# sinamalakouti/CDDMSL

Hardware: AMD Instinct MI355X
Metric: images/sec (train step) VOC+Clipart RN50-C4 (higher is better)
Workload: dtype bf16

## Files before the change

cddmsl_amd/csrc/conv_fwd.hip:

```cpp
#include "gemm_common.h"

namespace {

template <typename T> __device__ __forceinline__ void load8(const char* p, float* f);
template <> __device__ __forceinline__ void load8<__bf16>(const char* p, float* f) {
  const u32x4 v = *(const u32x4*)p;
#pragma unroll
  for (int j = 0; j < 4; ++j) { f[2 * j] = bf2f(v[j] & 0xffff); f[2 * j + 1] = bf2f(v[j] >> 16); }
}
template <> __device__ __forceinline__ void load8<float>(const char* p, float* f) {
  const f32x4 a = ((const f32x4*)p)[0], b = ((const f32x4*)p)[1];
  f[0] = a[0]; f[1] = a[1]; f[2] = a[2]; f[3] = a[3]; f[4] = b[0]; f[5] = b[1]; f[6] = b[2]; f[7] = b[3];
}

__device__ __forceinline__ int swz(int row, int chunk) { return row * KCH + (chunk ^ ((row >> 1) & 7)); }

template <typename T>
__global__ __launch_bounds__(256, 2) void k_conv_fwd_reg(ConvArgs p) {
  __shared__ __attribute__((aligned(16))) u32x4 lds[2][BM * KCH];
  const int t = threadIdx.x;
  const int ntn = (p.Cout + BN - 1) / BN;
  const int tile_n = blockIdx.x % ntn, tile_m = blockIdx.x / ntn;
  const int m0 = tile_m * BM, n0 = tile_n * BN;
  const int cc = t & 7, rb = t >> 3;
// ... 403 lines not shown
            }
#pragma unroll
            for (int j = 0; j < 8; ++j) v[j] += rv[j];
          }
          if (p.relu) {
#pragma unroll
            for (int j = 0; j < 8; ++j) v[j] = fmaxf(v[j], 0.f);
          }
          if (p.relu_mask) {
            float mv[8];
            if (PRE) {
#pragma unroll
              for (int j = 0; j < 4; ++j) { mv[2 * j] = bf2f(rmsk[a][i][j] & 0xffff); mv[2 * j + 1] = bf2f(rmsk[a][i][j] >> 16); }
            } else load8<T>(p.relu_mask + ((long)m * p.ldm + n) * Mma<T>::ES, mv);
#pragma unroll
            for (int j = 0; j < 8; ++j) if (!(mv[j] > 0.f)) v[j] = 0.f;
          }
          if (p.out_f32 || Mma<T>::ES == 4) {
            f32x4* dst = (f32x4*)(p.y + ((long)m * p.ldy + n) * 4);
            f32x4 o0 = {v[0], v[1], v[2], v[3]}, o1 = {v[4], v[5], v[6], v[7]};
            dst[0] = o0; dst[1] = o1;
          } else {
            u32x4 o = {pack2bf(v[0], v[1]), pack2bf(v[2], v[3]), pack2bf(v[4], v[5]), pack2bf(v[6], v[7])};
            *(u32x4*)(p.y + ((long)m * p.ldy + n) * 2) = o;
          }
        }
      }
    }
    return;
  }
#pragma unroll
  for (int b = 0; b < 2; ++b) {
    int n = n0 + wn * 64 + b * 32 + r;
    if (n >= p.Cout) continue;
    float sc = p.scale ? p.scale[n] : 1.f;
    float bi = p.bias ? p.bias[n] : 0.f;
#pragma unroll
    for (int a = 0; a < 2; ++a) {
#pragma unroll
      for (int g = 0; g < 16; ++g) {
        int m = m0 + wm * 64 + a * 32 + (g & 3) + 8 * (g >> 2) + 4 * h;
        if (m >= p.M) continue;
        float v = affine<T>(acc[a][b][g], sc, bi);
        if (p.residual) v += Mma<T>::load(p.residual + ((long)m * p.ldr + n) * Mma<T>::ES);
        if (p.relu) v = fmaxf(v, 0.f);
        if (p.relu_mask && !(Mma<T>::load(p.relu_mask + ((long)m * p.ldm + n) * Mma<T>::ES) > 0.f)) v = 0.f;
        if (p.out_f32) *(float*)(p.y + ((long)m * p.ldy + n) * 4) = v;
        else Mma<T>::store(p.y + ((long)m * p.ldy + n) * Mma<T>::ES, v);
      }
    }
  }
}

template <typename T, int CPP, int NT, int NTAP = 9>
__global__ __launch_bounds__(256) void k_conv3x3_small(ConvArgs p) {
  constexpr int KC = NTAP * CPP, KS = (KC + 1) / 2;
  constexpr int PAD = NTAP == 9 ? 1 : 0;
  constexpr int ES = Mma<T>::ES;
  const int lane = threadIdx.x & 63, r = lane & 31, hh = lane >> 5;
  constexpr bool WLDS = CPP > 1;
  __shared__ __attribute__((aligned(16))) u32x4 wl[WLDS ? NT * KS * 64 : 1];
  u32x4 bw[WLDS ? 1 : NT][WLDS ? 1 : KS];
  {
    const int wv = threadIdx.x >> 6;
#pragma unroll
    for (int nt = 0; nt < NT; ++nt)
#pragma unroll
      for (int ks = 0; ks < KS; ++ks) {
        if (WLDS && ((nt * KS + ks) & 3) != wv) continue;
        const int q = 2 * ks + hh;
        u32x4 v = {0u, 0u, 0u, 0u};
        if (q < KC) v = *(const u32x4*)(p.w + ((long)(nt * 32 + r) * KC + q) * 16);
        if (WLDS) wl[(nt * KS + ks) * 64 + lane] = v;
        else bw[WLDS ? 0 : nt][WLDS ? 0 : ks] = v;
      }
    if (WLDS) __syncthreads();
  }
  float sc[NT], bi[NT];
#pragma unroll
  for (int nt = 0; nt < NT; ++nt) { sc[nt] = p.scale ? p.scale[nt * 32 + r] : 1.f; bi[nt] = p.bias ? p.bias[nt * 32 + r] : 0.f; }
  const int wave = (blockIdx.x * blockDim.x + threadIdx.x) >> 6, nwaves = (gridDim.x * blockDim.x) >> 6;
  const int ntiles = (p.M + 31) >> 5;
  const __amdgpu_buffer_rsrc_t rx = __builtin_amdgcn_make_buffer_rsrc((void*)(p.x - (long)(p.Wi + 1) * (CPP * 16)), 0, 0x7fffffff, 0x00020000);
  const long ybytes = (long)p.M * p.ldy * ES, mbytes = (long)p.M * p.ldm * ES;
  const __amdgpu_buffer_rsrc_t ry = __builtin_amdgcn_make_buffer_rsrc((void*)p.y, 0, (int)(ybytes > 0x7fffffffL ? 0x7fffffffL : ybytes), 0x00020000);
  const __amdgpu_buffer_rsrc_t rm = __builtin_amdgcn_make_buffer_rsrc((void*)p.relu_mask, 0, p.relu_mask ? (int)(mbytes > 0x7fffffffL ? 0x7fffffffL : mbytes) : 0, 0x00020000);
  const float relu_floor = p.relu ? 0.f : -__builtin_inff();
  __shared__ __attribute__((aligned(16))) u32x4 ost[ES == 2 ? 4 * 32 * NT * 4 : 1];
  const bool ost_ok = !p.relu_mask && p.ldy == NT * 32 && (long)p.M * NT * 64 < 0x7fffffffL;
  for (int tile = wave; tile < ntiles; tile += nwaves) {
    const int m = tile * 32 + r;
    const bool vm = m < p.M;
    const unsigned mm = vm ? m : 0;
    const unsigned tq = fdiv(mm, p.dWo), ox = mm - tq * p.Wo;
    const unsigned img = fdiv(tq, p.dHo), oy = tq - img * p.Ho;
    const int iy0 = (int)oy * p.stride - PAD, ix0 = (int)ox * p.stride - PAD;
    const unsigned lbase = (unsigned)((((int)img * p.Hi + iy0 + 1) * p.Wi + ix0 + 1) * (CPP * 16)) + (CPP > 1 ? hh * 16 : 0);
    unsigned bad = vm ? 0u : 0x1ffu;
    if (NTAP == 9) {
#pragma unroll
      for (int ky = 0; ky < 3; ++ky)
#pragma unroll
        for (int kx = 0; kx < 3; ++kx)
          if ((unsigned)(iy0 + ky) >= (unsigned)p.Hi || (unsigned)(ix0 + kx) >= (unsigned)p.Wi) bad |= 1u << (3 * ky + kx);
    }
    u32x4 a[KS];
#pragma unroll
    for (int ks = 0; ks < KS; ++ks) {
      const int q0 = 2 * ks, q1 = 2 * ks + 1;
      const int t0 = q0 / CPP, c0 = q0 % CPP, t1 = q1 / CPP, c1 = q1 % CPP;
      if (CPP > 1) {
        const unsigned v = lbase | (__builtin_amdgcn_ubfe(bad, (unsigned)t0, 1u) << 31);
        a[ks] = __builtin_amdgcn_raw_buffer_load_b128(rx, v, ((t0 / 3) * p.Wi + (t0 % 3)) * (CPP * 16) + c0 * 16, 0);
      } else {
        const int ky = hh ? t1 / 3 : t0 / 3, kx = hh ? t1 % 3 : t0 % 3, cc = hh ? c1 : c0;
        const bool inq = hh ? (q1 < KC) : (q0 < KC);
        const int iy = iy0 + ky, ix = ix0 + kx;
        const bool ok = vm && inq && (unsigned)iy < (unsigned)p.Hi && (unsigned)ix < (unsigned)p.Wi;
        u32x4 v = {0u, 0u, 0u, 0u};
        if (ok) v = *(const u32x4*)(p.x + ((((long)img * p.Hi + iy0) * p.Wi + ix0) + (long)ky * p.Wi + kx) * (CPP * 16) + cc * 16);
        a[ks] = v;
      }
    }
    f32x16 acc[NT];
#pragma unroll
    for (int nt = 0; nt < NT; ++nt)
#pragma unroll
      for (int g = 0; g < 16; ++g) acc[nt][g] = 0.f;
    int wlane = lane;
    asm volatile("" : "+v"(wlane));
#pragma unroll
    for (int ks = 0; ks < KS; ++ks)
#pragma unroll
      for (int nt = 0; nt < NT; ++nt) {
        if (WLDS) Mma<T>::step(acc[nt], a[ks], wl[(nt * KS + ks) * 64 + wlane]);
        else Mma<T>::step(acc[nt], a[ks], bw[WLDS ? 0 : nt][WLDS ? 0 : ks]);
      }
    if (ES == 2 && ost_ok) {
      char* ob = (char*)ost + (threadIdx.x >> 6) * (32 * NT * 64);
#pragma unroll
      for (int nt = 0; nt < NT; ++nt)
#pragma unroll
        for (int g = 0; g < 16; ++g) {
          const int row = (g & 3) + 8 * (g >> 2) + 4 * hh;
          float v = affine<T>(acc[nt][g], sc[nt], bi[nt]);
          asm("v_max_f32 %0, %1, %2" : "=v"(v) : "v"(v), "s"(relu_floor));
          *(unsigned short*)(ob + row * (NT * 64) + (nt * 32 + r) * 2) = f2bf(v);
        }
#pragma unroll
      for (int i = 0; i < 2 * NT; ++i) {
        const u32x4 o = *(const u32x4*)(ob + (i * 64 + lane) * 16);
        __builtin_amdgcn_raw_buffer_store_b128(o, ry, (unsigned)((i * 64 + lane) * 16), tile * (32 * NT * 64), 0);
      }
      continue;
    }
    const unsigned vy = (unsigned)(((tile * 32 + 4 * hh) * p.ldy + r) * ES), vmk = (unsigned)(((tile * 32 + 4 * hh) * p.ldm + r) * ES);
#pragma unroll
    for (int nt = 0; nt < NT; ++nt)
#pragma unroll
      for (int g = 0; g < 16; ++g) {
        const int row = (g & 3) + 8 * (g >> 2);
        float v = affine<T>(acc[nt][g], sc[nt], bi[nt]);
        asm("v_max_f32 %0, %1, %2" : "=v"(v) : "v"(v), "s"(relu_floor));
        if (p.relu_mask) {
          float mv;
          if (ES == 2) mv = bf2f((unsigned)__builtin_amdgcn_raw_buffer_load_b16(rm, vmk, (row * p.ldm + nt * 32) * ES, 0));
          else mv = __builtin_bit_cast(float, __builtin_amdgcn_raw_buffer_load_b32(rm, vmk, (row * p.ldm + nt * 32) * ES, 0));
          if (!(mv > 0.f)) v = 0.f;
        }
        if (ES == 2) __builtin_amdgcn_raw_buffer_store_b16((unsigned short)f2bf(v), ry, vy, (row * p.ldy + nt * 32) * ES, 0);
        else __builtin_amdgcn_raw_buffer_store_b32(__builtin_bit_cast(unsigned, v), ry, vy, (row * p.ldy + nt * 32) * ES, 0);
      }
  }
}

template <typename T> void launch_small(const ConvArgs& a, unsigned nb, hipStream_t st) {
  if (a.KH == 1 && a.cpp == 8) hipLaunchKernelGGL((k_conv3x3_small<T, 8, 2, 1>), dim3(nb), dim3(256), 0, st, a);
  else if (a.KH == 1) hipLaunchKernelGGL((k_conv3x3_small<T, 32, 2, 1>), dim3(nb), dim3(256), 0, st, a);
  else if (a.cpp == 1 && a.Cout == 32) hipLaunchKernelGGL((k_conv3x3_small<T, 1, 1>), dim3(nb), dim3(256), 0, st, a);
  else if (a.cpp == 1) hipLaunchKernelGGL((k_conv3x3_small<T, 1, 2>), dim3(nb), dim3(256), 0, st, a);
  else if (a.cpp == 8) hipLaunchKernelGGL((k_conv3x3_small<T, 8, 2>), dim3(nb), dim3(256), 0, st, a);
  else if (a.Cout == 32) hipLaunchKernelGGL((k_conv3x3_small<T, 4, 1>), dim3(nb), dim3(256), 0, st, a);
  else hipLaunchKernelGGL((k_conv3x3_small<T, 4, 2>), dim3(nb), dim3(256), 0, st, a);
}

template <typename T> void launch_tile128(const ConvArgs& a, const Plan& p, hipStream_t st) {
  const dim3 grid(p.gx, p.gy);
  switch (p.kernel) {
    case 8: launch_small<T>(a, p.gx, st); break;
    case 2: hipLaunchKernelGGL(k_conv_fwd_reg<T>, grid, dim3(256), 0, st, a); break;
    default: hipLaunchKernelGGL(k_conv_fwd<T>, grid, dim3(256), 0, st, a); break;
  }
}

}

void launch_fwd_tile128(const ConvArgs& a, const Plan& p, Operand op, hipStream_t st) {
  if (op == OP_BF16) launch_tile128<__bf16>(a, p, st);
  else launch_tile128<float>(a, p, st);
}
```

cddmsl_amd/csrc/elementwise.hip:

```cpp
#include "common.h"
#include <stdlib.h>

namespace {

template <typename T> struct Elt;
template <> struct Elt<__bf16> {
  static constexpr int ES = 2, VEC = 8;
  __device__ static __forceinline__ void unpack(const u32x4& v, float* f) {
#pragma unroll
    for (int j = 0; j < 4; ++j) { f[2 * j] = bf2f(v[j] & 0xffff); f[2 * j + 1] = bf2f(v[j] >> 16); }
  }
  __device__ static __forceinline__ u32x4 pack(const float* f) {
    u32x4 v;
#pragma unroll
    for (int j = 0; j < 4; ++j) v[j] = pack2bf(f[2 * j], f[2 * j + 1]);
    return v;
  }
  __device__ static __forceinline__ float ld(const char* p) { return bf2f(*(const unsigned short*)p); }
  __device__ static __forceinline__ void st(char* p, float v) { *(unsigned short*)p = f2bf(v); }
};
template <> struct Elt<float> {
  static constexpr int ES = 4, VEC = 4;
  __device__ static __forceinline__ void unpack(const u32x4& v, float* f) {
    const f32x4 x = __builtin_bit_cast(f32x4, v);
// ... 90 lines not shown
                                int RH, int RW, int top, int left, int S, int Cp,
                                float m0, float m1, float m2, float s0, float s1, float s2) {
  preprocess224_px<T>(img, out, n, h, w, Hp, Wp, RH, RW, top, left, S, Cp, m0, m1, m2, s0, s1, s2);
}
template <typename T>
__global__ void k_preprocess224_batch(PreBatch b, char* out, int n0, int Hp, int Wp, int RH, int RW, int top, int left, int S, int Cp,
                                      float m0, float m1, float m2, float s0, float s1, float s2) {
  const int j = blockIdx.y;
  preprocess224_px<T>(b.img[j], out, n0 + j, b.h[j], b.w[j], Hp, Wp, RH, RW, top, left, S, Cp, m0, m1, m2, s0, s1, s2);
}

template <typename T>
__global__ void k_avgpool2_fwd(const char* x, char* y, int N, int H, int W, int cch) {
  int Ho = H / 2, Wo = W / 2;
  long total = (long)N * Ho * Wo * cch;
  for (long i = (long)blockIdx.x * blockDim.x + threadIdx.x; i < total; i += (long)gridDim.x * blockDim.x) {
    int c = i % cch; long q = i / cch;
    int ox = q % Wo; q /= Wo;
    int oy = q % Ho; int n = q / Ho;
    const u32x4* b = (const u32x4*)x + (((long)n * H + 2 * oy) * W + 2 * ox) * cch + c;
    float a0[8], a1[8], a2[8], a3[8], o[8];
    Elt<T>::unpack(b[0], a0); Elt<T>::unpack(b[cch], a1);
    Elt<T>::unpack(b[(long)W * cch], a2); Elt<T>::unpack(b[(long)W * cch + cch], a3);
#pragma unroll
    for (int j = 0; j < Elt<T>::VEC; ++j) o[j] = ((a0[j] + a1[j]) + (a2[j] + a3[j])) * 0.25f;
    ((u32x4*)y)[i] = Elt<T>::pack(o);
  }
}

template <typename T>
__global__ void k_avgpool2_bwd(const char* dy, const char* mask, const char* add, char* dx, int N, int H, int W, int cch) {
  int Ho = H / 2, Wo = W / 2;
  long total = (long)N * H * W * cch;
  for (long i = (long)blockIdx.x * blockDim.x + threadIdx.x; i < total; i += (long)gridDim.x * blockDim.x) {
    int c = i % cch; long q = i / cch;
    int xx = q % W; q /= W;
    int yy = q % H; int n = q / H;
    float g[8], m[8], a[8], o[8];
    bool in = (yy >> 1) < Ho && (xx >> 1) < Wo;
    if (in) Elt<T>::unpack(((const u32x4*)dy)[(((long)n * Ho + (yy >> 1)) * Wo + (xx >> 1)) * cch + c], g);
    if (mask) Elt<T>::unpack(((const u32x4*)mask)[i], m);
    if (add) Elt<T>::unpack(((const u32x4*)add)[i], a);
#pragma unroll
    for (int j = 0; j < Elt<T>::VEC; ++j) {
      float v = in ? g[j] * 0.25f : 0.f;
      if (add) v += a[j];
      if (mask && !(m[j] > 0.f)) v = 0.f;
      o[j] = v;
    }
    ((u32x4*)dx)[i] = Elt<T>::pack(o);
  }
}

__global__ __launch_bounds__(256) void k_avgpool2_bwd_q8(const char* dy, const char* mask, const char* add, char* dx, int N, int H, int W, int cch,
                                                         char* y8, const float* q8, unsigned* amax8) {
  using T = __bf16;
  const int Ho = H / 2, Wo = W / 2;
  const long total = (long)N * H * W * cch;
  const float s = q8[0];
  unsigned mx = 0u;
  for (long i = (long)blockIdx.x * blockDim.x + threadIdx.x; i < total; i += (long)gridDim.x * blockDim.x) {
    int c = i % cch; long q = i / cch;
    int xx = q % W; q /= W;
    int yy = q % H; int n = q / H;
    float g[8], m[8], a[8], o[8];
    bool in = (yy >> 1) < Ho && (xx >> 1) < Wo;
    if (in) Elt<T>::unpack(((const u32x4*)dy)[(((long)n * Ho + (yy >> 1)) * Wo + (xx >> 1)) * cch + c], g);
    if (mask) Elt<T>::unpack(((const u32x4*)mask)[i], m);
    if (add) Elt<T>::unpack(((const u32x4*)add)[i], a);
#pragma unroll
    for (int j = 0; j < 8; ++j) {
      float v = in ? g[j] * 0.25f : 0.f;
      if (add) v += a[j];
      if (mask && !(m[j] > 0.f)) v = 0.f;
      o[j] = v;
      mx = absmax_bits(mx, v);
    }
    ((u32x4*)dx)[i] = Elt<T>::pack(o);
    const u32x2 o8 = {e4m3x4(o[0] * s, o[1] * s, o[2] * s, o[3] * s), e4m3x4(o[4] * s, o[5] * s, o[6] * s, o[7] * s)};
    ((u32x2*)y8)[i] = o8;
  }
  __shared__ unsigned sm[4];
  mx = wave_max_u(mx);
  if ((threadIdx.x & 63) == 0) sm[threadIdx.x >> 6] = mx;
  __syncthreads();
  if (threadIdx.x == 0) {
    const unsigned a = sm[0] > sm[1] ? sm[0] : sm[1], b = sm[2] > sm[3] ? sm[2] : sm[3];
    atomicMax(amax8 + (blockIdx.x & 63), a > b ? a : b);
  }
}

template <typename T>
__global__ void k_maxpool3s2(const char* x, char* y, int N, int H, int W, int Ho, int Wo, int cch) {
  long total = (long)N * Ho * Wo * cch;
  for (long i = (long)blockIdx.x * blockDim.x + threadIdx.x; i < total; i += (long)gridDim.x * blockDim.x) {
    int c = i % cch; long q = i / cch;
    int ox = q % Wo; q /= Wo;
    int oy = q % Ho; int n = q / Ho;
    float m[8], v[8];
#pragma unroll
    for (int j = 0; j < 8; ++j) m[j] = -INFINITY;
    for (int dy = 0; dy < 3; ++dy) {
      int iy = 2 * oy - 1 + dy;
      if (iy < 0 || iy >= H) continue;
      for (int dx = 0; dx < 3; ++dx) {
        int ix = 2 * ox - 1 + dx;
// ... 376 lines not shown
extern "C" int cddmsl_preprocess_batch(const unsigned char* const* imgs, const int* hs, const int* ws, int N, void* out, int Hp, int Wp,
                                       int Cp, const float* mean3, const float* std3, int div255, int dtype, void* stream) {
  if (N < 0 || Cp < 3 || !imgs || !hs || !ws) return CDDMSL_ERR_ARG;
  for (int j = 0; j < N; ++j) if (hs[j] <= 0 || ws[j] <= 0 || hs[j] > Hp || ws[j] > Wp || !imgs[j]) return CDDMSL_ERR_ARG;
  hipStream_t st = (hipStream_t)stream;
  const long px = (long)Hp * Wp;
  for (int n0 = 0; n0 < N; n0 += PRE_MAX) {
    const int c = N - n0 < PRE_MAX ? N - n0 : PRE_MAX;
    PreBatch b;
    for (int j = 0; j < PRE_MAX; ++j) { const int q = j < c ? j : 0; b.img[j] = imgs[n0 + q]; b.h[j] = hs[n0 + q]; b.w[j] = ws[n0 + q]; }
    DISPATCH(dtype, k_preprocess_batch, <<<dim3((unsigned)((px + 255) / 256), (unsigned)c), dim3(256), 0, st>>>(
        b, (char*)out, n0, Hp, Wp, Cp, mean3[0], mean3[1], mean3[2], std3[0], std3[1], std3[2], div255 ? 255.0f : 1.0f));
  }
  return launch_status();
}
extern "C" int cddmsl_preprocess224_batch(const unsigned char* const* imgs, const int* hs, const int* ws, int N, void* out, int Hp, int Wp,
                                          int RH, int RW, int top, int left, int S, int Cp, const float* mean3, const float* std3,
                                          int dtype, void* stream) {
  if (N < 0 || Cp < 3 || !imgs || !hs || !ws || S <= 0 || top < 0 || left < 0 || top + S > RH || left + S > RW) return CDDMSL_ERR_ARG;
  for (int j = 0; j < N; ++j) if (hs[j] <= 0 || ws[j] <= 0 || hs[j] > Hp || ws[j] > Wp || !imgs[j]) return CDDMSL_ERR_ARG;
  hipStream_t st = (hipStream_t)stream;
  for (int n0 = 0; n0 < N; n0 += PRE_MAX) {
    const int c = N - n0 < PRE_MAX ? N - n0 : PRE_MAX;
    PreBatch b;
    for (int j = 0; j < PRE_MAX; ++j) { const int q = j < c ? j : 0; b.img[j] = imgs[n0 + q]; b.h[j] = hs[n0 + q]; b.w[j] = ws[n0 + q]; }
    DISPATCH(dtype, k_preprocess224_batch, <<<dim3((unsigned)((S * S + 255) / 256), (unsigned)c), dim3(256), 0, st>>>(
        b, (char*)out, n0, Hp, Wp, RH, RW, top, left, S, Cp, mean3[0], mean3[1], mean3[2], std3[0], std3[1], std3[2]));
  }
  return launch_status();
}

extern "C" int cddmsl_avgpool2_fwd(const void* x, void* y, int N, int H, int W, int C, int dtype, void* stream) {
  int es = dtype == 0 ? 2 : 4;
  if ((C * es) % 16 || H < 2 || W < 2) return CDDMSL_ERR_ARG;
  int cch = C * es / 16;
  long total = (long)N * (H / 2) * (W / 2) * cch;
  if (total == 0) return CDDMSL_OK;
  DISPATCH(dtype, k_avgpool2_fwd, <<<dim3(gsz(total)), dim3(256), 0, (hipStream_t)stream>>>((const char*)x, (char*)y, N, H, W, cch));
  return launch_status();
}

extern "C" int cddmsl_avgpool2_bwd(const void* dy, const void* mask, const void* add, void* dx, int N, int H, int W,
                                   int C, int dtype, void* stream) {
  int es = dtype == 0 ? 2 : 4;
  if ((C * es) % 16 || H < 2 || W < 2) return CDDMSL_ERR_ARG;
  int cch = C * es / 16;
  long total = (long)N * H * W * cch;
  if (total == 0) return CDDMSL_OK;
  DISPATCH(dtype, k_avgpool2_bwd, <<<dim3(gsz(total)), dim3(256), 0, (hipStream_t)stream>>>(
      (const char*)dy, (const char*)mask, (const char*)add, (char*)dx, N, H, W, cch));
  return launch_status();
}

extern "C" int cddmsl_avgpool2_bwd_q8(const void* dy, const void* mask, const void* add, void* dx, int N, int H, int W, int C, void* y8,
                                      const float* q8, float* amax8, void* stream) {
  if ((C * 2) % 16 || !y8 || !q8 || !amax8) return CDDMSL_ERR_ARG;
  const int cch = C * 2 / 16;
  const long total = (long)N * H * W * cch;
  if (total == 0) return CDDMSL_OK;
  hipLaunchKernelGGL(k_avgpool2_bwd_q8, dim3(gsz(total, 256, 8192)), dim3(256), 0, (hipStream_t)stream, (const char*)dy, (const char*)mask, (const char*)add,
                     (char*)dx, N, H, W, cch, (char*)y8, q8, (unsigned*)amax8);
  return launch_status();
}

extern "C" int cddmsl_maxpool3s2_fwd(const void* x, void* y, int N, int H, int W, int C, int dtype, void* stream) {
  int es = dtype == 0 ? 2 : 4;
  if ((C * es) % 16 || H < 1 || W < 1) return CDDMSL_ERR_ARG;
  int cch = C * es / 16, Ho = (H - 1) / 2 + 1, Wo = (W - 1) / 2 + 1;
  long total = (long)N * Ho * Wo * cch;
  if (total == 0) return CDDMSL_OK;
  DISPATCH(dtype, k_maxpool3s2, <<<dim3(gsz(total)), dim3(256), 0, (hipStream_t)stream>>>((const char*)x, (char*)y, N, H, W, Ho, Wo, cch));
  return launch_status();
}
extern "C" int cddmsl_upsample_zero2(const void* t, const void* mask, const void* add, void* dx, int N, int H, int W, int C,
                                     int dtype, void* stream) {
  int es = dtype == 0 ? 2 : 4;
  if ((C * es) % 16 || H < 1 || W < 1) return CDDMSL_ERR_ARG;
  int cch = C * es / 16, Ho = (H - 1) / 2 + 1, Wo = (W - 1) / 2 + 1;
  long total = (long)N * H * W * cch;
  if (total == 0) return CDDMSL_OK;
  DISPATCH(dtype, k_upsample_zero2, <<<dim3(gsz(total)), dim3(256), 0, (hipStream_t)stream>>>(
      (const char*)t, (const char*)mask, (const char*)add, (char*)dx, N, H, W, Ho, Wo, cch));
  return launch_status();
}
extern "C" int cddmsl_meanpool_fwd(const void* x, float* y, long K, int P, int C, int dtype, void* stream) {
  if (K < 0 || P <= 0 || C <= 0) return CDDMSL_ERR_ARG;
  if (K == 0) return CDDMSL_OK;
  long n = K * C;
  DISPATCH(dtype, k_meanpool_fwd, <<<dim3((unsigned)((n + 255) / 256)), dim3(256), 0, (hipStream_t)stream>>>((const char*)x, y, K, P, C));
  return launch_status();
}
extern "C" int cddmsl_meanpool_bwd(const float* dy, void* dx, long K, int P, int C, int dtype, void* stream) {
  if (K < 0 || P <= 0 || C <= 0) return CDDMSL_ERR_ARG;
  if (K == 0) return CDDMSL_OK;
  long n = K * P * C;
  DISPATCH(dtype, k_meanpool_bwd, <<<dim3((unsigned)((n + 255) / 256)), dim3(256), 0, (hipStream_t)stream>>>(dy, (char*)dx, K, P, C));
  return launch_status();
}

extern "C" int cddmsl_attn_tokens_fwd(const void* x, const float* pos, void* tok, int K, int P, int TP, int C, int dtype, void* stream) {
  int es = dtype == 0 ? 2 : 4;
  if ((C * es) % 16 || P <= 0 || TP < P + 1) return CDDMSL_ERR_ARG;
  int cch = C * es / 16;
  long total = (long)K * cch;
  if (total == 0) return CDDMSL_OK;
  DISPATCH(dtype, k_attn_tokens_fwd, <<<dim3(gsz(total, 64)), dim3(64), 0, (hipStream_t)stream>>>((const char*)x, pos, (char*)tok, nullptr, K, P, TP, cch));
// ... 102 lines not shown
```

cddmsl_amd/csrc/gemm_common.h:

```cpp
#pragma once
#include "common.h"
#include <cstdlib>

namespace {

constexpr int BM = 128, BN = 128, KCH = 8;

struct FastDiv {
  unsigned mul, shr, d;
};
static inline FastDiv make_fastdiv(unsigned d) {
  FastDiv f;
  f.d = d;
  unsigned s = 0;
  while ((1ull << s) < d) ++s;
  f.shr = s;
  f.mul = (unsigned)(((1ull << 32) * ((1ull << s) - d)) / d + 1);
  return f;
}
__device__ __forceinline__ unsigned fdiv(unsigned n, const FastDiv& f) { return (__umulhi(n, f.mul) + n) >> f.shr; }

template <typename T> __device__ __forceinline__ float affine(float v, float sc, float bi) {
  return sizeof(T) <= 2 ? __builtin_fmaf(v, sc, bi) : v * sc + bi;
}

#ifndef CDDMSL_STORE_AUX
#define CDDMSL_STORE_AUX 2
#endif
#ifndef CDDMSL_LOAD_AUX
#define CDDMSL_LOAD_AUX 0
#endif

struct ConvArgs {
  const char* x;
  const char* w;
  char* y;
  const float* scale;
  const float* bias;
  const char* residual;
  const char* relu_mask;
  int Nimg, Hi, Wi, Cin, Ho, Wo, Cout, KH, KW, stride, pad;
  int ldy, ldr, ldm;
  int relu, out_f32, pool;
  int res_f32;
  int res_pool;
  int M, Kc, cpp;
  FastDiv dWo, dHo, dcpp, dKW;
  int xrs, wrs;
  long bx, bw, by;
  char* y8 = nullptr;
  const float* q8 = nullptr;
  unsigned* amax8 = nullptr;
  float* partial = nullptr;
  int tile0 = 0, ksplits = 1, kper = 0, tile_limit = 0;
  int nt_out = 1;
#ifdef CDDMSL_TILE_STAMPS
  unsigned long long* tstamps = nullptr;
#endif
};

template <typename T> struct Mma;
template <> struct Mma<__bf16> {
  static constexpr int ES = 2;
  __device__ static __forceinline__ void step(f32x16& acc, const u32x4& a, const u32x4& b) {
    acc = __builtin_amdgcn_mfma_f32_32x32x16_bf16(__builtin_bit_cast(bf16x8, a), __builtin_bit_cast(bf16x8, b), acc, 0, 0, 0);
  }
  __device__ static __forceinline__ float load(const char* p) { return bf2f(*(const unsigned short*)p); }
  __device__ static __forceinline__ void store(char* p, float v) { *(unsigned short*)p = f2bf(v); }
};
template <> struct Mma<float> {
  static constexpr int ES = 4;
  __device__ static __forceinline__ void step(f32x16& acc, const u32x4& a, const u32x4& b) {
    const f32x4 fa = __builtin_bit_cast(f32x4, a), fb = __builtin_bit_cast(f32x4, b);
    acc = __builtin_amdgcn_mfma_f32_32x32x2f32(fa[0], fb[0], acc, 0, 0, 0);
    acc = __builtin_amdgcn_mfma_f32_32x32x2f32(fa[1], fb[1], acc, 0, 0, 0);
    acc = __builtin_amdgcn_mfma_f32_32x32x2f32(fa[2], fb[2], acc, 0, 0, 0);
    acc = __builtin_amdgcn_mfma_f32_32x32x2f32(fa[3], fb[3], acc, 0, 0, 0);
  }
  __device__ static __forceinline__ float load(const char* p) { return *(const float*)p; }
  __device__ static __forceinline__ void store(char* p, float v) { *(float*)p = v; }
};
typedef __attribute__((ext_vector_type(8))) int i32x8;

__device__ __forceinline__ int xcd_remap(int bid, int nblk) {
  const int q = nblk >> 3, rem = nblk & 7, x = bid & 7, j = bid >> 3;
  return (x < rem ? x * (q + 1) : rem * (q + 1) + (x - rem) * q) + j;
}

template <typename T> __device__ __forceinline__ u32x4 avg4(const u32x4& a, const u32x4& b, const u32x4& c, const u32x4& d);
template <> __device__ __forceinline__ u32x4 avg4<float>(const u32x4& a, const u32x4& b, const u32x4& c, const u32x4& d) {
  const f32x4 fa = __builtin_bit_cast(f32x4, a), fb = __builtin_bit_cast(f32x4, b);
  const f32x4 fc = __builtin_bit_cast(f32x4, c), fd = __builtin_bit_cast(f32x4, d);
  f32x4 r = ((fa + fb) + (fc + fd)) * 0.25f;
  return __builtin_bit_cast(u32x4, r);
}
template <> __device__ __forceinline__ u32x4 avg4<__bf16>(const u32x4& a, const u32x4& b, const u32x4& c, const u32x4& d) {
  u32x4 r;
#pragma unroll
  for (int j = 0; j < 4; ++j) {
    float lo = (bf2f(a[j] & 0xffff) + bf2f(b[j] & 0xffff)) + (bf2f(c[j] & 0xffff) + bf2f(d[j] & 0xffff));
    float hi = (bf2f(a[j] >> 16) + bf2f(b[j] >> 16)) + (bf2f(c[j] >> 16) + bf2f(d[j] >> 16));
    r[j] = pack2bf(lo * 0.25f, hi * 0.25f);
  }
  return r;
}

__device__ __attribute__((aligned(16))) unsigned int g_zero_page[4] = {0u, 0u, 0u, 0u};
// ... 83 lines not shown
```

cddmsl_amd/csrc/gemm_conv.hip:

```cpp
#include "gemm_common.h"

namespace {

template <typename T>
__device__ __forceinline__ void weight_prep_body(const float* w, const float* scale, char* wf, char* wd, int Cout, int KH, int KW, int Cin,
                                                 long first, long stride) {
  __shared__ float tile[32][33];
  const int taps = KH * KW, nit = (Cin + 31) / 32, nct = (Cout + 31) / 32;
  const long ntiles = (long)nct * taps * nit;
  const int tx = threadIdx.x & 31, ty = threadIdx.x >> 5;
  constexpr int ES = Mma<T>::ES;
  for (long tl = first; tl < ntiles; tl += stride) {
    const int it = (int)(tl % nit); const long q = tl / nit;
    const int tap = (int)(q % taps), ct = (int)(q / taps);
    const int ky = tap / KW, kx = tap % KW;
    __syncthreads();
#pragma unroll
    for (int r = 0; r < 4; ++r) {
      const int co = ct * 32 + ty + 8 * r, ci = it * 32 + tx;
      float v = 0.f;
      if (co < Cout && ci < Cin) {
        const long i = ((long)co * taps + tap) * Cin + ci;
        v = w[i];
        if (wf) Mma<T>::store(wf + i * ES, v);
// ... 117 lines not shown
  if ((Cin * es) % 16 != 0) return CDDMSL_ERR_ARG;
  if (pool && (KH != 1 || KW != 1 || pad != 0 || stride != 1)) return CDDMSL_ERR_ARG;
  a.x = (const char*)x; a.w = (const char*)w; a.y = (char*)y; a.scale = scale; a.bias = bias;
  a.residual = (const char*)residual; a.relu_mask = (const char*)relu_mask;
  a.Nimg = Nimg; a.Hi = Hi; a.Wi = Wi; a.Cin = Cin; a.Cout = Cout; a.KH = KH; a.KW = KW; a.stride = stride; a.pad = pad;
  if (pool) { a.Ho = Hi / 2; a.Wo = Wi / 2; }
  else { a.Ho = (Hi + 2 * pad - KH) / stride + 1; a.Wo = (Wi + 2 * pad - KW) / stride + 1; }
  if (a.Ho <= 0 || a.Wo <= 0) return CDDMSL_ERR_ARG;
  if ((out_f32 & 2) && (!(out_f32 & 1) || !residual || relu_mask || pool)) return CDDMSL_ERR_ARG;
  a.ldy = ldy; a.ldr = ldr; a.ldm = ldm; a.relu = relu; a.out_f32 = out_f32 & 1; a.pool = pool;
  a.res_f32 = (op == OP_BF16 && (out_f32 & 2)) ? 1 : 0;
  a.res_pool = (out_f32 & 4) ? 1 : 0;
  if (a.res_pool && (!residual || (out_f32 & 2) || pool || KH != 1 || KW != 1 || pad != 0 || (long)Nimg * (a.Ho / 2) * (a.Wo / 2) * ldr * es >= (1L << 31) ||
                     (Cout & 7) || (ldy & 7) || (ldr & 7) || (relu_mask && (ldm & 7)))) return CDDMSL_ERR_ARG;
  if (a.res_f32 && ((Cout & 7) || (ldy & 7) || (ldr & 7))) return CDDMSL_ERR_ARG;
  long M = (long)Nimg * a.Ho * a.Wo;
  if (M > 0x7fffff00L) return CDDMSL_ERR_ARG;
  a.M = (int)M; a.cpp = Cin * es / 16; a.Kc = KH * KW * a.cpp;
  a.dWo = make_fastdiv((unsigned)a.Wo); a.dHo = make_fastdiv((unsigned)a.Ho);
  a.dcpp = make_fastdiv((unsigned)a.cpp); a.dKW = make_fastdiv((unsigned)KW);
  a.xrs = a.cpp; a.wrs = a.Kc; a.bx = a.bw = a.by = 0;
#ifdef CDDMSL_TILE_STAMPS
  a.tstamps = g_tile_stamps;
#endif
  if (a.M == 0) return CDDMSL_OK;
  a.nt_out = nt_out_for((long)a.M * Cout * 2);
  if (y8) {
    if (op == OP_F32 || (out_f32 & 1) || ldy != Cout) return CDDMSL_ERR_ARG;
    a.y8 = (char*)y8; a.q8 = q8; a.amax8 = (unsigned*)amax8;
  }
  return CDDMSL_OK;
}

static int conv_fwd_any(Operand op, const void* x, const void* w, void* y, const float* scale, const float* bias,
                        const void* residual, const void* relu_mask, int Nimg, int Hi, int Wi, int Cin,
                        int Cout, int KH, int KW, int stride, int pad, int pool, int ldy, int ldr, int ldm,
                        int relu, int out_f32, void* y8, const float* q8, float* amax8, void* stream) {
  ConvArgs a;
  const int st = fill_conv(a, op, x, w, y, scale, bias, residual, relu_mask, Nimg, Hi, Wi, Cin, Cout, KH, KW, stride, pad, pool, ldy, ldr, ldm,
                           relu, out_f32, y8, q8, amax8);
  if (st != CDDMSL_OK || a.M == 0) return st;
  return run_fwd(a, op, plan_fwd(a, op, 1), stream);
}

extern "C" int cddmsl_conv_fwd(const void* x, const void* w, void* y, const float* scale, const float* bias,
                               const void* residual, const void* relu_mask, int Nimg, int Hi, int Wi, int Cin,
                               int Cout, int KH, int KW, int stride, int pad, int pool, int ldy, int ldr, int ldm,
                               int relu, int out_f32, int dtype, void* stream) {
  if (dtype != 0 && dtype != 1) return CDDMSL_ERR_ARG;
  return conv_fwd_any((Operand)dtype, x, w, y, scale, bias, residual, relu_mask, Nimg, Hi, Wi, Cin, Cout, KH, KW, stride, pad, pool, ldy, ldr, ldm,
                      relu, out_f32, nullptr, nullptr, nullptr, stream);
}

extern "C" int cddmsl_conv_fwd_q8(const void* x, const void* w, void* y, const float* scale, const float* bias,
                                  const void* residual, const void* relu_mask, int Nimg, int Hi, int Wi, int Cin,
                                  int Cout, int KH, int KW, int stride, int pad, int relu, void* y8, const float* q8, float* amax8,
                                  void* stream) {
  if (!y8) return CDDMSL_ERR_ARG;
  return conv_fwd_any(OP_BF16, x, w, y, scale, bias, residual, relu_mask, Nimg, Hi, Wi, Cin, Cout, KH, KW, stride, pad, 0, Cout, Cout, Cout,
                      relu, 0, y8, q8, amax8, stream);
}

extern "C" int cddmsl_conv_fwd_fp8(const void* x, const void* w, void* y, const float* scale, const float* bias,
                                   const void* residual, const void* relu_mask, int Nimg, int Hi, int Wi, int Cin, int Cout, int KH,
                                   int KW, int pad, int relu, int out_f32, void* y8, const float* q8, float* amax8, void* stream) {
  if (Cin % 128 != 0 || (out_f32 & ~1)) return CDDMSL_ERR_ARG;
  return conv_fwd_any(OP_FP8, x, w, y, scale, bias, residual, relu_mask, Nimg, Hi, Wi, Cin, Cout, KH, KW, 1, pad, 0, Cout, Cout, Cout,
                      relu, out_f32, y8, q8, amax8, stream);
}

static bool wgrad256_ok(const WgradArgs& a, int batch) {
  const long mode = env_int("CDDMSL_GEMM256", 1);
  if (mode == 0) return false;
  if ((a.Cout & 255) || (a.K & 255) || (a.cpp & 7) || (a.ldd & 7)) return false;
  if (mode == 2) return true;
  return (long)(a.Cout / 256) * (a.K / 256) * batch * ((a.M + WM - 1) / WM) >= env_int("CDDMSL_WGRAD256_MIN", 4000);
}
static bool wgrad256_span_ok(int mtiles_per_split, int Wi, long row_bytes) {
  return ((long)mtiles_per_split * WM + WM + 2L * Wi + 2) * row_bytes + (1L << 20) < (1L << 31);
}

static int even_split(int total_mt, long* splits) {
  const int mps = (int)((total_mt + *splits - 1) / *splits);
  *splits = (total_mt + mps - 1) / mps;
  return mps;
}

static long split_512_rounds(long tiles, int total_mt, bool taps) {
  bool forced;
  const long target = env_int("CDDMSL_WGRAD_BLOCKS", taps ? 1024 : 512, &forced);
  const long maxs = (total_mt + 7) / 8;
  long splits = 1;
  const long r0 = (target + 511) / 512;
  double best = -1.0;
  for (long r = r0; r <= r0 + 1; ++r) {
    long c = (512 * r) / tiles;
    if (c < 1) c = 1;
    if (c > maxs) c = maxs;
    long real = c;
    even_split(total_mt, &real);
    const long blocks = tiles * real, rounds = (blocks + 511) / 512;
    const double eff = (double)blocks / (512.0 * rounds);
    if (eff > best + 0.03) { best = eff; splits = c; }
    if (c == maxs) break;
  }
  if (forced) { splits = (target + tiles - 1) / tiles; if (splits > maxs) splits = maxs; }
// ... 219 lines not shown
```

cddmsl_amd/csrc/losses.hip:

```cpp
#include "common.h"

namespace {

__device__ __forceinline__ float block_sum(float v, float* red) {
  v = wave_sum(v);
  __syncthreads();
  if ((threadIdx.x & 63) == 0) red[threadIdx.x >> 6] = v;
  __syncthreads();
  float s = 0.f;
  for (int i = 0; i < (int)(blockDim.x >> 6); ++i) s += red[i];
  return s;
}
__device__ __forceinline__ float block_max(float v, float* red) {
  v = wave_max(v);
  __syncthreads();
  if ((threadIdx.x & 63) == 0) red[threadIdx.x >> 6] = v;
  __syncthreads();
  float s = -INFINITY;
  for (int i = 0; i < (int)(blockDim.x >> 6); ++i) s = fmaxf(s, red[i]);
  return s;
}

__global__ void k_l2norm_fwd(const float* x, float* y, float* inv, int D, float eps) {
  __shared__ float red[4];
// ... 148 lines not shown
  long tot = (long)n * n;
  k_contrastive_grad<<<dim3((unsigned)((tot + 255) / 256)), dim3(256), 0, (hipStream_t)stream>>>(S, rlse, clse, gloss, dS, n, ld);
  return launch_status();
}

namespace {

template <typename T> struct OutT;
template <> struct OutT<__bf16> { __device__ static __forceinline__ void st(void* p, long i, float v) { ((unsigned short*)p)[i] = f2bf(v); }
                                  __device__ static __forceinline__ float ld(const void* p, long i) { return bf2f(((const unsigned short*)p)[i]); } };
template <> struct OutT<float> { __device__ static __forceinline__ void st(void* p, long i, float v) { ((float*)p)[i] = v; }
                                 __device__ static __forceinline__ float ld(const void* p, long i) { return ((const float*)p)[i]; } };
__device__ __forceinline__ void st4(__bf16*, void* p, long i4, float4 v) { ((uint2*)p)[i4] = make_uint2(pack2bf(v.x, v.y), pack2bf(v.z, v.w)); }
__device__ __forceinline__ void st4(float*, void* p, long i4, float4 v) { ((float4*)p)[i4] = v; }
__device__ __forceinline__ float4 ld4(__bf16*, const void* p, long i4) {
  const uint2 u = ((const uint2*)p)[i4];
  return make_float4(__uint_as_float(u.x << 16), __uint_as_float(u.x & 0xffff0000u), __uint_as_float(u.y << 16), __uint_as_float(u.y & 0xffff0000u));
}
__device__ __forceinline__ float4 ld4(float*, const void* p, long i4) { return ((const float4*)p)[i4]; }

template <typename T, int NSEG>
__global__ __launch_bounds__(256) void k_layernorm_fwd_v(const float* __restrict__ x, const float* __restrict__ gamma,
                                                         const float* __restrict__ beta, void* __restrict__ y, float* __restrict__ mean,
                                                         float* __restrict__ rstd, long R, float eps) {
  constexpr int D = NSEG * 256;
  const long r = (long)blockIdx.x * 4 + (threadIdx.x >> 6);
  const int lane = threadIdx.x & 63;
  if (r >= R) return;
  const float4* xr = (const float4*)(x + r * D);
  float4 v[NSEG];
#pragma unroll
  for (int s = 0; s < NSEG; ++s) v[s] = xr[s * 64 + lane];
  float sum = 0.f;
#pragma unroll
  for (int s = 0; s < NSEG; ++s) sum += (v[s].x + v[s].y) + (v[s].z + v[s].w);
  const float mu = wave_sum(sum) / (float)D;
  float var = 0.f;
#pragma unroll
  for (int s = 0; s < NSEG; ++s) {
    const float a = v[s].x - mu, b = v[s].y - mu, c = v[s].z - mu, d = v[s].w - mu;
    var += (a * a + b * b) + (c * c + d * d);
  }
  const float rs = rsqrtf(wave_sum(var) / (float)D + eps);
#pragma unroll
  for (int s = 0; s < NSEG; ++s) {
    const float4 g = ((const float4*)gamma)[s * 64 + lane], b = ((const float4*)beta)[s * 64 + lane];
    float4 o;
    o.x = (v[s].x - mu) * rs * g.x + b.x; o.y = (v[s].y - mu) * rs * g.y + b.y;
    o.z = (v[s].z - mu) * rs * g.z + b.z; o.w = (v[s].w - mu) * rs * g.w + b.w;
    st4((T*)nullptr, y, r * (D / 4) + s * 64 + lane, o);
  }
  if (lane == 0) { mean[r] = mu; rstd[r] = rs; }
}
template <typename T, int NSEG>
__global__ __launch_bounds__(256) void k_layernorm_bwd_v(const void* __restrict__ dy, const float* __restrict__ x,
                                                         const float* __restrict__ gamma, const float* __restrict__ mean,
                                                         const float* __restrict__ rstd, float* dx, long R, int accumulate) {
  constexpr int D = NSEG * 256;
  const long r = (long)blockIdx.x * 4 + (threadIdx.x >> 6);
  const int lane = threadIdx.x & 63;
  if (r >= R) return;
  const float4* xr = (const float4*)(x + r * D);
  float4* dxr = (float4*)(dx + r * D);
  const float mu = mean[r], rs = rstd[r];
  float4 g[NSEG], xh[NSEG], o[NSEG];
#pragma unroll
  for (int s = 0; s < NSEG; ++s) {
    const float4 d4 = ld4((T*)nullptr, dy, r * (D / 4) + s * 64 + lane), ga = ((const float4*)gamma)[s * 64 + lane], xv = xr[s * 64 + lane];
    if (accumulate) o[s] = dxr[s * 64 + lane];
    g[s] = make_float4(d4.x * ga.x, d4.y * ga.y, d4.z * ga.z, d4.w * ga.w);
    xh[s] = make_float4((xv.x - mu) * rs, (xv.y - mu) * rs, (xv.z - mu) * rs, (xv.w - mu) * rs);
  }
  float sg = 0.f, sgx = 0.f;
#pragma unroll
  for (int s = 0; s < NSEG; ++s) {
    sg += (g[s].x + g[s].y) + (g[s].z + g[s].w);
    sgx += (g[s].x * xh[s].x + g[s].y * xh[s].y) + (g[s].z * xh[s].z + g[s].w * xh[s].w);
  }
  sg = wave_sum(sg) / (float)D; sgx = wave_sum(sgx) / (float)D;
#pragma unroll
  for (int s = 0; s < NSEG; ++s) {
    float4 v;
    v.x = rs * (g[s].x - sg - xh[s].x * sgx); v.y = rs * (g[s].y - sg - xh[s].y * sgx);
    v.z = rs * (g[s].z - sg - xh[s].z * sgx); v.w = rs * (g[s].w - sg - xh[s].w * sgx);
    if (accumulate) { v.x = o[s].x + v.x; v.y = o[s].y + v.y; v.z = o[s].z + v.z; v.w = o[s].w + v.w; }
    dxr[s * 64 + lane] = v;
  }
}
template <typename T> bool layernorm_fwd_v(const float* x, const float* gamma, const float* beta, void* y, float* mean, float* rstd,
                                           long R, int D, float eps, hipStream_t st) {
  const dim3 grid((unsigned)((R + 3) / 4)), blk(256);
  switch (D) {
    case 256: k_layernorm_fwd_v<T, 1><<<grid, blk, 0, st>>>(x, gamma, beta, y, mean, rstd, R, eps); return true;
    case 512: k_layernorm_fwd_v<T, 2><<<grid, blk, 0, st>>>(x, gamma, beta, y, mean, rstd, R, eps); return true;
    case 768: k_layernorm_fwd_v<T, 3><<<grid, blk, 0, st>>>(x, gamma, beta, y, mean, rstd, R, eps); return true;
    case 1024: k_layernorm_fwd_v<T, 4><<<grid, blk, 0, st>>>(x, gamma, beta, y, mean, rstd, R, eps); return true;
  }
  return false;
}
template <typename T> bool layernorm_bwd_v(const void* dy, const float* x, const float* gamma, const float* mean, const float* rstd,
                                           float* dx, long R, int D, int accumulate, hipStream_t st) {
  const dim3 grid((unsigned)((R + 3) / 4)), blk(256);
  switch (D) {
    case 256: k_layernorm_bwd_v<T, 1><<<grid, blk, 0, st>>>(dy, x, gamma, mean, rstd, dx, R, accumulate); return true;
    case 512: k_layernorm_bwd_v<T, 2><<<grid, blk, 0, st>>>(dy, x, gamma, mean, rstd, dx, R, accumulate); return true;
    case 768: k_layernorm_bwd_v<T, 3><<<grid, blk, 0, st>>>(dy, x, gamma, mean, rstd, dx, R, accumulate); return true;
    case 1024: k_layernorm_bwd_v<T, 4><<<grid, blk, 0, st>>>(dy, x, gamma, mean, rstd, dx, R, accumulate); return true;
  }
  return false;
}
__host__ inline bool aligned16(const void* a, const void* b, const void* c, const void* d, const void* e = nullptr) {
  return ((((size_t)a) | ((size_t)b) | ((size_t)c) | ((size_t)d) | ((size_t)e)) & 15) == 0;
}

template <typename T>
__global__ void k_layernorm_fwd(const float* x, const float* gamma, const float* beta, void* y, float* mean, float* rstd,
                                long R, int D, float eps) {
  long r = (long)blockIdx.x * 4 + (threadIdx.x >> 6);
  int lane = threadIdx.x & 63;
  if (r >= R) return;
  const float* xr = x + r * D;
  float s = 0.f;
  for (int d = lane; d < D; d += 64) s += xr[d];
  float mu = wave_sum(s) / (float)D;
  float v = 0.f;
  for (int d = lane; d < D; d += 64) { float c = xr[d] - mu; v += c * c; }
  float rs = rsqrtf(wave_sum(v) / (float)D + eps);
  for (int d = lane; d < D; d += 64) OutT<T>::st(y, r * D + d, (xr[d] - mu) * rs * gamma[d] + beta[d]);
  if (lane == 0) { mean[r] = mu; rstd[r] = rs; }
}
template <typename T>
__global__ void k_layernorm_bwd(const void* dy, const float* x, const float* gamma, const float* mean, const float* rstd,
                                float* dx, long R, int D, int accumulate) {
  long r = (long)blockIdx.x * 4 + (threadIdx.x >> 6);
  int lane = threadIdx.x & 63;
  if (r >= R) return;
  const float* xr = x + r * D;
  float mu = mean[r], rs = rstd[r];
  float sg = 0.f, sgx = 0.f;
  for (int d = lane; d < D; d += 64) {
    float g = OutT<T>::ld(dy, r * D + d) * gamma[d];
    float xh = (xr[d] - mu) * rs;
    sg += g; sgx += g * xh;
  }
  sg = wave_sum(sg) / (float)D; sgx = wave_sum(sgx) / (float)D;
  for (int d = lane; d < D; d += 64) {
    float g = OutT<T>::ld(dy, r * D + d) * gamma[d];
    float xh = (xr[d] - mu) * rs;
    float v = rs * (g - sg - xh * sgx);
    dx[r * D + d] = accumulate ? dx[r * D + d] + v : v;
  }
}

__global__ void k_focal_ce_fwd(const float* logits, const long* target, float* row_loss, float* probs, long R, int C,
                               float gamma, int bg_class, float bg_weight) {
// ... 10 lines not shown
  float zt = __shfl(z, t, 64), pt = __shfl(p, t, 64);
  if (lane == 0) {
    float ce = (mx + logf(se)) - zt;
    float w = (t == bg_class) ? bg_weight : 1.f;
    float mod = gamma > 0.f ? powf(fmaxf(1.f - pt, 0.f), gamma) : 1.f;
    row_loss[r] = ce * mod * w;
  }
}
__global__ void k_focal_ce_bwd(const float* logits, const long* target, const float* probs, const float* gscale, float* dlogits,
                               long R, int C, float gamma, int bg_class, float bg_weight) {
  long r = (long)blockIdx.x * 4 + (threadIdx.x >> 6);
  int lane = threadIdx.x & 63;
  if (r >= R) return;
  int t = (int)target[r];
  float p = lane < C ? probs[r * C + lane] : 0.f;
  float pt = __shfl(p, t, 64);
  float w = (t == bg_class) ? bg_weight : 1.f;
  float one = lane == t ? 1.f : 0.f;
  float ce = -logf(fmaxf(pt, 1e-38f));
  float omp = fmaxf(1.f - pt, 0.f);
  float mod = gamma > 0.f ? powf(omp, gamma) : 1.f;
  float dmod = (gamma > 0.f && omp > 0.f) ? -gamma * powf(omp, gamma - 1.f) * pt * (one - p) : 0.f;
  float g = w * (mod * (p - one) + ce * dmod) * gscale[0];
  if (lane < C) dlogits[r * C + lane] = g;
}

}

extern "C" int cddmsl_layernorm_fwd(const float* x, const float* gamma, const float* beta, void* y, float* mean, float* rstd,
                                    long R, int D, float eps, int dtype, void* stream) {
  if (R < 0 || D <= 0 || (dtype != 0 && dtype != 1)) return CDDMSL_ERR_ARG;
  if (R == 0) return CDDMSL_OK;
  dim3 grid((unsigned)((R + 3) / 4));
  if (aligned16(x, gamma, beta, y) &&
      (dtype == 0 ? layernorm_fwd_v<__bf16>(x, gamma, beta, y, mean, rstd, R, D, eps, (hipStream_t)stream)
                  : layernorm_fwd_v<float>(x, gamma, beta, y, mean, rstd, R, D, eps, (hipStream_t)stream)))
    return launch_status();
  if (dtype == 0) k_layernorm_fwd<__bf16><<<grid, dim3(256), 0, (hipStream_t)stream>>>(x, gamma, beta, y, mean, rstd, R, D, eps);
  else k_layernorm_fwd<float><<<grid, dim3(256), 0, (hipStream_t)stream>>>(x, gamma, beta, y, mean, rstd, R, D, eps);
  return launch_status();
}
extern "C" int cddmsl_layernorm_bwd(const void* dy, const float* x, const float* gamma, const float* mean, const float* rstd,
                                    float* dx, long R, int D, int accumulate, int dtype, void* stream) {
  if (R < 0 || D <= 0 || (dtype != 0 && dtype != 1)) return CDDMSL_ERR_ARG;
  if (R == 0) return CDDMSL_OK;
  dim3 grid((unsigned)((R + 3) / 4));
  if (aligned16(dy, x, gamma, dx) &&
      (dtype == 0 ? layernorm_bwd_v<__bf16>(dy, x, gamma, mean, rstd, dx, R, D, accumulate, (hipStream_t)stream)
                  : layernorm_bwd_v<float>(dy, x, gamma, mean, rstd, dx, R, D, accumulate, (hipStream_t)stream)))
    return launch_status();
  if (dtype == 0) k_layernorm_bwd<__bf16><<<grid, dim3(256), 0, (hipStream_t)stream>>>(dy, x, gamma, mean, rstd, dx, R, D, accumulate);
  else k_layernorm_bwd<float><<<grid, dim3(256), 0, (hipStream_t)stream>>>(dy, x, gamma, mean, rstd, dx, R, D, accumulate);
  return launch_status();
}
extern "C" int cddmsl_focal_ce_fwd(const float* logits, const long* target, float* row_loss, float* probs, long R, int C,
                                   float gamma, int bg_class, float bg_weight, void* stream) {
  if (R < 0 || C <= 0 || C > 64) return CDDMSL_ERR_ARG;
  if (R == 0) return CDDMSL_OK;
  k_focal_ce_fwd<<<dim3((unsigned)((R + 3) / 4)), dim3(256), 0, (hipStream_t)stream>>>(logits, target, row_loss, probs, R, C, gamma, bg_class, bg_weight);
  return launch_status();
}
extern "C" int cddmsl_focal_ce_bwd(const float* logits, const long* target, const float* probs, const float* gscale,
                                   float* dlogits, long R, int C, float gamma, int bg_class, float bg_weight, void* stream) {
  if (R < 0 || C <= 0 || C > 64) return CDDMSL_ERR_ARG;
  if (R == 0) return CDDMSL_OK;
  k_focal_ce_bwd<<<dim3((unsigned)((R + 3) / 4)), dim3(256), 0, (hipStream_t)stream>>>(logits, target, probs, gscale, dlogits, R, C, gamma, bg_class, bg_weight);
  return launch_status();
}

namespace {
struct BoxW { float wx, wy, ww, wh; };
__device__ __forceinline__ void get_deltas4(const float* s, const float* t, BoxW w, float* d) {
  const float sw = s[2] - s[0], sh = s[3] - s[1];
  const float sx = s[0] + 0.5f * sw, sy = s[1] + 0.5f * sh;
  const float tw = t[2] - t[0], th = t[3] - t[1];
  const float tx = t[0] + 0.5f * tw, ty = t[1] + 0.5f * th;
  d[0] = w.wx * (tx - sx) / sw; d[1] = w.wy * (ty - sy) / sh;
  d[2] = w.ww * logf(tw / sw); d[3] = w.wh * logf(th / sh);
}
__device__ __forceinline__ float sgn(float v) { return v > 0.f ? 1.f : (v < 0.f ? -1.f : 0.f); }

__global__ __launch_bounds__(256) void k_rpn_losses(const float* logits, const float* deltas, const long* pos, int npos, const long* neg, int nneg,
                                                     const long* midx, const float* gt, const long* gt_off, const float* anchors, long A, BoxW w,
                                                     float inv_norm, float* out2, const float* gout2, float* dlogits, float* ddeltas) {
  __shared__ float red[4];
  const bool bwd = gout2 != nullptr;
  const float gc = bwd ? gout2[0] * inv_norm : 0.f, gl = bwd ? gout2[1] * inv_norm : 0.f;
  float cls = 0.f, loc = 0.f;
  for (int i = threadIdx.x; i < npos + nneg; i += blockDim.x) {
    const bool is_pos = i < npos;
    const long r = is_pos ? pos[i] : neg[i - npos];
    const float x = logits[r], y = is_pos ? 1.f : 0.f;
    if (!bwd) cls += fmaxf(x, 0.f) - x * y + log1pf(expf(-fabsf(x)));
    else dlogits[r] = (1.f / (1.f + expf(-x)) - y) * gc;
    if (is_pos) {
      const long img = r / A, a = r - img * A;
      float d[4];
      get_deltas4(anchors + 4 * a, gt + 4 * (midx[r] + gt_off[img]), w, d);
#pragma unroll
      for (int c = 0; c < 4; ++c) {
        const float e = deltas[4 * r + c] - d[c];
        if (!bwd) loc += fabsf(e); else ddeltas[4 * r + c] = sgn(e) * gl;
      }
    }
  }
  if (!bwd) {
// ... 46 lines not shown
```

cddmsl_amd/hip.py:

```python
import ctypes
import os
from ctypes import c_float, c_int, c_long, c_void_p

import torch

from ._lib import check, lib, ptr, require_cuda, stream_ptr

DT = {torch.bfloat16: 0, torch.float32: 1}

_sigs_done = False


def _L():
    global _sigs_done
    L = lib()
    if not _sigs_done:
        vp, ci, cf = c_void_p, c_int, c_float
        L.cddmsl_last_kernel.argtypes = []
        L.cddmsl_plan_only.argtypes = [ci]
        L.cddmsl_conv_fwd.argtypes = [vp] * 7 + [ci] * 16 + [vp]
        L.cddmsl_bottleneck64_ok.argtypes = [ci] * 4
        L.cddmsl_bottleneck64_fwd.argtypes = [vp] * 17 + [ci] * 4 + [vp]
        L.cddmsl_conv_wgrad.argtypes = [vp] * 4 + [ci] * 12 + [vp]
        L.cddmsl_set_workspace.argtypes = [vp, c_long]
        L.cddmsl_weight_prep.argtypes = [vp] * 4 + [ci] * 5 + [vp]
        L.cddmsl_weight_prep_multi.argtypes = [vp, ci, ci, vp]
        L.cddmsl_preprocess.argtypes = [vp, vp] + [ci] * 6 + [vp, vp, ci, ci, vp]
        L.cddmsl_maxpool3s2_fwd.argtypes = [vp, vp] + [ci] * 5 + [vp]
        L.cddmsl_upsample_zero2.argtypes = [vp] * 4 + [ci] * 5 + [vp]
        L.cddmsl_meanpool_fwd.argtypes = [vp, vp, c_long, ci, ci, ci, vp]
        L.cddmsl_meanpool_bwd.argtypes = [vp, vp, c_long, ci, ci, ci, vp]
        L.cddmsl_preprocess224.argtypes = [vp, vp] + [ci] * 11 + [vp, vp, ci, vp]
        L.cddmsl_preprocess_batch.argtypes = [vp, vp, vp, ci, vp, ci, ci, ci, vp, vp, ci, ci, vp]
        L.cddmsl_preprocess224_batch.argtypes = [vp, vp, vp, ci, vp] + [ci] * 8 + [vp, vp, ci, vp]
        L.cddmsl_avgpool2_fwd.argtypes = [vp, vp] + [ci] * 5 + [vp]
        L.cddmsl_avgpool2_bwd.argtypes = [vp] * 4 + [ci] * 5 + [vp]
        L.cddmsl_avgpool2_bwd_q8.argtypes = [vp] * 4 + [ci] * 4 + [vp] * 4
        L.cddmsl_attn_tokens_fwd.argtypes = [vp] * 3 + [ci] * 5 + [vp]
        L.cddmsl_attn_tokens_bwd.argtypes = [vp] * 4 + [ci] * 5 + [vp]
        L.cddmsl_attnpool_softmax_fwd.argtypes = [vp] * 3 + [c_long, ci, ci, ci, cf, ci, vp]
        L.cddmsl_attnpool_softmax_bwd.argtypes = [vp] * 4 + [c_long, ci, ci, ci, cf, ci, vp]
        L.cddmsl_gemm_nt_batched.argtypes = [vp] * 4 + [ci] * 7 + [c_long] * 3 + [ci, ci, vp]
        L.cddmsl_gemm_tn_batched.argtypes = [vp] * 3 + [ci] * 7 + [c_long] * 3 + [ci, ci, vp]
        L.cddmsl_relu_bwd.argtypes = [vp, vp, vp, c_long, ci, ci, vp]
        L.cddmsl_colsum.argtypes = [vp, vp, c_long, ci, ci, ci, vp]
        L.cddmsl_sgd_clip_step.argtypes = [vp] * 4 + [ci, vp] + [cf] * 4 + [ci, vp]
        L.cddmsl_roi_align_forward.argtypes = [vp] * 5 + [ci] * 7 + [cf, ci, ci, ci, vp]
        L.cddmsl_roi_align_backward.argtypes = [vp] * 7 + [ci] * 7 + [cf, ci, ci, ci, vp]
        L.cddmsl_nms_anyorder.argtypes = [vp] * 4 + [ci, cf, vp, vp, vp]
        L.cddmsl_roi_align_nchw_anyorder.argtypes = [vp] * 3 + [ci] * 7 + [cf, ci, ci, ci, vp, vp, vp]
        L.cddmsl_roi_align_backward_nchw_anyorder.argtypes = [vp] * 3 + [ci] * 7 + [cf, ci, ci, ci, vp, vp, vp]
        L.cddmsl_quantize_fp8.argtypes = [vp] * 4 + [c_long, ci, vp]
        L.cddmsl_conv_fwd_fp8.argtypes = [vp] * 7 + [ci] * 10 + [vp] * 4
        L.cddmsl_conv_wgrad_fp8_ok.argtypes = [ci] * 6
        L.cddmsl_conv_wgrad_fp8.argtypes = [vp] * 4 + [ci] * 9 + [vp]
        L.cddmsl_conv_fwd_q8.argtypes = [vp] * 7 + [ci] * 10 + [vp] * 4
        L.cddmsl_fp8_dot_nt.argtypes = [vp] * 4 + [ci] * 4 + [vp]
        L.cddmsl_roi_align_forward_affine.argtypes = [vp] * 6 + [ci] * 8 + [cf, ci, ci, ci] + [vp] * 4
        L.cddmsl_roi_align_backward_pooled.argtypes = [vp] * 7 + [ci] * 7 + [cf, ci, ci, ci, vp]
        L.cddmsl_anchors.argtypes = [vp, vp, ci, ci, ci, cf, cf, vp]
        L.cddmsl_sort_desc.argtypes = [vp] * 5 + [ci, ci, vp, vp, vp]
        L.cddmsl_rpn_decode.argtypes = [vp] * 6 + [ci] * 5 + [cf] * 8 + [vp]
        L.cddmsl_nms.argtypes = [vp] * 5 + [ci, ci, cf, ci, vp]
        L.cddmsl_iou_match.argtypes = [vp, ci, vp, ci, vp, vp, vp, ci, cf, cf, ci, ci, ci, ci, vp]
        L.cddmsl_iou_match_batched.argtypes = [vp] * 7 + [ci] * 5 + [cf, cf] + [ci] * 4 + [vp]
        L.cddmsl_l2norm_fwd.argtypes = [vp, vp, vp, c_long, ci, cf, vp]
        L.cddmsl_l2norm_bwd.argtypes = [vp, vp, vp, vp, c_long, ci, vp]
        L.cddmsl_cosine_logits_fwd.argtypes = [vp] * 4 + [c_long, ci, ci, cf, cf, vp]
        L.cddmsl_cosine_logits_bwd.argtypes = [vp] * 5 + [c_long, ci, ci, cf, ci, vp]
        L.cddmsl_layernorm_fwd.argtypes = [vp] * 6 + [c_long, ci, cf, ci, vp]
        L.cddmsl_layernorm_bwd.argtypes = [vp] * 6 + [c_long, ci, ci, ci, vp]
        L.cddmsl_focal_ce_fwd.argtypes = [vp] * 4 + [c_long, ci, cf, ci, cf, vp]
        L.cddmsl_focal_ce_bwd.argtypes = [vp] * 5 + [c_long, ci, cf, ci, cf, vp]
        L.cddmsl_attn_small_fwd.argtypes = [vp] * 4 + [ci] * 8 + [cf, ci, vp]
        L.cddmsl_attn_small_bwd.argtypes = [vp] * 7 + [ci] * 8 + [cf, ci, vp]
        L.cddmsl_attn_tokens_fwd_mask.argtypes = [vp] * 4 + [ci] * 5 + [vp]
        L.cddmsl_attnpool_dx.argtypes = [vp] * 6 + [ci] * 6 + [vp]
        L.cddmsl_rpn_losses.argtypes = [vp, vp, vp, ci, vp, ci, vp, vp, vp, vp, c_long, cf, cf, cf, cf, cf, vp, vp, vp, vp, vp]
        L.cddmsl_box_l1.argtypes = [vp, ci, vp, ci, vp, vp, vp, cf, cf, cf, cf, cf, vp, vp, vp, vp]
        L.cddmsl_attn_last_fwd.argtypes = [vp] * 4 + [ci] * 8 + [cf, ci, vp]
        L.cddmsl_attn_last_bwd.argtypes = [vp] * 6 + [ci] * 8 + [cf, ci, vp]
        L.cddmsl_contrastive_fwd.argtypes = [vp] * 4 + [ci, ci, vp]
        L.cddmsl_contrastive_bwd.argtypes = [vp] * 5 + [ci, ci, vp]
        L.cddmsl_instance_boxes.argtypes = [vp] + [ci] * 4 + [vp, ci, vp, vp, vp, vp]
        L.cddmsl_text_embed.argtypes = [vp] * 4 + [c_long, ci, ci, ci, ci, vp]
        L.cddmsl_attn_causal_fwd.argtypes = [vp, vp] + [ci] * 6 + [cf, ci, vp]
        L.cddmsl_quick_gelu.argtypes = [vp, c_long, ci, vp]
        L.cddmsl_text_pool.argtypes = [vp] * 5 + [c_long, ci, ci, ci, cf, ci, vp]
        L.cddmsl_skinny_gemm_workspace.argtypes = [ci] * 3
        L.cddmsl_skinny_gemm.argtypes = [vp] * 6 + [c_long] + [ci] * 4 + [vp]
        L.cddmsl_lm_head_workspace.argtypes = [ci, ci]
        L.cddmsl_lm_head_argmax.argtypes = [vp, vp, vp, ci, vp, vp, c_long, ci, ci, ci, vp]
        L.cddmsl_decode_attn.argtypes = [vp] * 4 + [ci] * 6 + [cf, ci, vp]
        L.cddmsl_pos_embed.argtypes = [vp, ci] + [vp] * 4 + [c_long] + [ci] * 6 + [vp]
        L.cddmsl_gelu_new.argtypes = [vp, c_long, ci, vp]
        L.cddmsl_lm_head_topk_workspace.argtypes = [ci, ci]
        L.cddmsl_lm_head_topk.argtypes = [vp] * 7 + [c_long] + [ci] * 4 + [vp]
        L.cddmsl_beam_step.argtypes = [vp] * 15 + [ci] * 5 + [vp]
        L.cddmsl_decode_attn_beam.argtypes = [vp] * 7 + [ci] * 9 + [cf, ci, vp]
        _sigs_done = True
    return L


class _Profiler:

    def __init__(self):
        self.on = False
        self.only = None
        self.events = []
        self.shapes = []

    def enable(self, only=None):
        self.on, self.only, self.events, self.shapes = True, (set(only) if only else None), [], []

    def begin(self, name=None, plan=None):
        if not self.on:
            return None
        if self.only is not None:
            if name is None and plan is not None:
                L = _L()
                L.cddmsl_plan_only(1)
                try:
                    plan()
                finally:
# ... 84 lines not shown
    N, H, W, Cin = x.shape
    Cout, KH, KW, Cin2 = w.shape
    assert Cin == Cin2, (x.shape, w.shape)
    if pool:
        Ho, Wo = H // 2, W // 2
    else:
        Ho, Wo = (H + 2 * pad - KH) // stride + 1, (W + 2 * pad - KW) // stride + 1
    ydt = torch.float32 if out_f32 else x.dtype
    if out_spec is not None and out_spec.full is None:
        out_spec.full = torch.empty((2 * N, Ho, Wo, Cout), device=x.device, dtype=ydt)
        y, out_spec.used = out_spec.full[:N], 1
    elif out_spec is not None and out_spec.used == 1 and tuple(out_spec.full.shape) == (2 * N, Ho, Wo, Cout) and out_spec.full.dtype == ydt:
        y, out_spec.used = out_spec.full[N:], 2
    else:
        y = torch.empty((N, Ho, Wo, Cout), device=x.device, dtype=ydt)
    for v in (scale, bias):
        assert v is None or (v.dtype == torch.float32 and v.numel() == Cout and v.is_contiguous())
    res_f32 = residual is not None and residual.dtype == torch.float32 and x.dtype != torch.float32
    if res_f32:
        assert out_f32 and relu_mask is None and not pool and Cout % 8 == 0
    if residual_pooled:
        assert residual is not None and not res_f32 and residual.dtype == x.dtype and residual.is_contiguous()
        assert tuple(residual.shape) == (N, Ho // 2, Wo // 2, Cout) and pooled_residual_ok(residual), residual.shape
    for v in (residual, relu_mask):
        assert v is None or (v is residual and residual_pooled) or (
            (v.dtype == x.dtype or (v is residual and res_f32)) and v.is_contiguous() and v.numel() == y.numel())
    y8 = None
    if emit8 is not None:
        assert x.dtype == torch.bfloat16 and not out_f32 and not pool and not residual_pooled and not res_f32
        y8 = torch.empty(y.shape, device=x.device, dtype=torch.uint8)

    def launch():
        if y8 is not None:
            return _L().cddmsl_conv_fwd_q8(ptr(x), ptr(w), ptr(y), ptr(scale), ptr(bias), ptr(residual), ptr(relu_mask),
                                           N, H, W, Cin, Cout, KH, KW, stride, pad, int(relu), ptr(y8), ptr(emit8[0]), ptr(emit8[1]), stream_ptr())
        return _L().cddmsl_conv_fwd(ptr(x), ptr(w), ptr(y), ptr(scale), ptr(bias), ptr(residual), ptr(relu_mask),
                                    N, H, W, Cin, Cout, KH, KW, stride, pad, int(pool), Cout, Cout, Cout,
                                    int(relu), int(out_f32) | (2 if res_f32 else 0) | (4 if residual_pooled else 0), _dt(x), stream_ptr())
    e0 = PROFILE.begin(plan=launch) if PROFILE.on else None
    st = launch()
    check(st, "cddmsl_conv_fwd")
    PROFILE.end(e0, _CONV_KERNEL.get(_L().cddmsl_last_kernel(), "conv_fwd") if e0 is not None else "conv_fwd",
                2.0 * N * Ho * Wo * Cout * KH * KW * Cin,
                (N * Ho * Wo, Cout, KH * KW * Cin, KH, int(pool), stride),
                nbytes=float(_conv_input_pixels(N, H, W, Ho, Wo, KH, KW, stride, bool(pool)) * Cin * x.element_size()
                             + w.numel() * w.element_size() + y.numel() * y.element_size()
                             + (residual.numel() * residual.element_size() if residual is not None else 0)
                             + (relu_mask.numel() * relu_mask.element_size() if relu_mask is not None else 0)))
    if y8 is not None:
        y._fp8 = (y8, emit8[0].data_ptr())
    return y


def bottleneck64_ok(o1, w2, w3, wd=None, w1n=None):
    if not (o1.is_cuda and o1.dtype == torch.bfloat16 and o1.dim() == 4 and o1.is_contiguous() and o1.shape[3] == 64):
        return False
    want = ((w2, (64, 3, 3, 64)), (w3, (256, 1, 1, 64)), (wd, (256, 1, 1, 64)), (w1n, (64, 1, 1, 256)))
    if any(w is not None and (tuple(w.shape) != s or w.dtype != torch.bfloat16 or not w.is_contiguous()) for w, s in want):
        return False
    N, H, W, _ = o1.shape
    return N > 0 and bool(_L().cddmsl_bottleneck64_ok(N, H, W, 0))


def bottleneck64_fwd(o1, w2, bn2, w3, bn3, residual=None, x0=None, wd=None, bnd=None, w1n=None, bn1n=None):
    require_cuda(o1, w2, w3, residual, x0, wd, w1n)
    assert bottleneck64_ok(o1, w2, w3, wd, w1n) and (residual is None) != (wd is None)
    N, H, W, _ = o1.shape
    for t, c in ((residual, 256), (x0 if wd is not None else None, 64)):
        assert t is None or (t.dtype == torch.bfloat16 and t.is_contiguous() and tuple(t.shape) == (N, H, W, c))
    for bn, c in ((bn2, 64), (bn3, 256), (bnd, 256), (bn1n, 64)):
        assert bn is None or all(v.dtype == torch.float32 and v.numel() == c and v.is_contiguous() and v.is_cuda for v in bn)
    assert (wd is None) == (bnd is None) and (w1n is None) == (bn1n is None) and (wd is None or x0 is not None)
    out = torch.empty((N, H, W, 256), device=o1.device, dtype=o1.dtype)
    o1n = torch.empty((N, H, W, 64), device=o1.device, dtype=o1.dtype) if w1n is not None else None
    sd, bd = bnd if bnd is not None else (None, None)
    s1n, b1n = bn1n if bn1n is not None else (None, None)
    e0 = PROFILE.begin(name="k_bottleneck64") if PROFILE.on else None
    check(_L().cddmsl_bottleneck64_fwd(ptr(o1), ptr(w2), ptr(bn2[0]), ptr(bn2[1]), ptr(w3), ptr(bn3[0]), ptr(bn3[1]), ptr(residual),
                                       ptr(x0 if wd is not None else None), ptr(wd), ptr(sd), ptr(bd), ptr(w1n), ptr(s1n), ptr(b1n),
                                       ptr(out), ptr(o1n), N, H, W, 0, stream_ptr()), "cddmsl_bottleneck64_fwd")
    M = N * H * W
    kn = 576 * 64 + 64 * 256 + (64 * 256 if wd is not None else 0) + (256 * 64 if w1n is not None else 0)
    PROFILE.end(e0, "k_bottleneck64", 2.0 * M * kn, (M, 256, 576, 3, int(wd is not None), int(w1n is not None)),
                nbytes=float(2 * M * (64 + (64 if wd is not None else 256) + 256 + (64 if w1n is not None else 0)) + 2 * kn))
    return out, o1n


def conv_emit8_ok(M, Cout, KH, KW, Cin_chunks_ok=True):
    return Cout % 256 == 0 and KH * KW <= 31 and ((M + 255) // 256) * (Cout // 256) >= 160 and Cin_chunks_ok and os.environ.get("CDDMSL_GEMM256", "1") != "0"


FP8_MAX = 448.0


@_timed("quantize_fp8")
def quantize_fp8(x, scale=None, amax=None):
    require_cuda(x, scale, amax)
    assert x.is_contiguous() and x.dtype in (torch.bfloat16, torch.float32) and x.numel() % 8 == 0
    y = torch.empty(x.shape, device=x.device, dtype=torch.uint8)
    check(_L().cddmsl_quantize_fp8(ptr(x), ptr(y), ptr(scale), ptr(amax), x.numel(), 0 if x.dtype == torch.bfloat16 else 1, stream_ptr()),
          "cddmsl_quantize_fp8")
    return y


def conv_fwd_fp8_ok(M, Cin, Cout, KH, KW, pad):
    min_tiles = int(os.environ.get("CDDMSL_FP8_MIN_TILES", "160"))
# ... 142 lines not shown
def _f3(v):
    return (c_float * 3)(*[float(x) for x in v])


def _image_table(images_u8):
    import ctypes
    n = len(images_u8)
    ptrs = (ctypes.c_void_p * n)(*[im.data_ptr() for im in images_u8])
    hs = (ctypes.c_int * n)(*[int(im.shape[1]) for im in images_u8])
    ws = (ctypes.c_int * n)(*[int(im.shape[2]) for im in images_u8])
    return ptrs, hs, ws


@_timed("preprocess")
def preprocess(images_u8, Hp, Wp, mean, std, dtype, Cp=None, div255=True):
    require_cuda(*images_u8)
    Cp = Cp or (8 if dtype == torch.bfloat16 else 4)
    out = torch.empty((len(images_u8), Hp, Wp, Cp), device=images_u8[0].device, dtype=dtype)
    m, s = _f3(mean), _f3(std)
    for im in images_u8:
        assert im.dtype == torch.uint8 and im.dim() == 3 and im.shape[0] == 3 and im.is_contiguous()
    ptrs, hs, ws = _image_table(images_u8)
    check(_L().cddmsl_preprocess_batch(ptrs, hs, ws, len(images_u8), ptr(out), Hp, Wp, Cp, m, s, int(div255), DT[dtype], stream_ptr()),
          "cddmsl_preprocess_batch")
    return out


@_timed("preprocess224")
def preprocess224(images_u8, Hp, Wp, mean, std, dtype, size=224, Cp=None):
    require_cuda(*images_u8)
    Cp = Cp or (8 if dtype == torch.bfloat16 else 4)
    if Wp <= Hp:
        RW, RH = size, int(size * Hp / Wp)
    else:
        RH, RW = size, int(size * Wp / Hp)
    top, left = int(round((RH - size) / 2.0)), int(round((RW - size) / 2.0))
    out = torch.empty((len(images_u8), size, size, Cp), device=images_u8[0].device, dtype=dtype)
    m, s = _f3(mean), _f3(std)
    for im in images_u8:
        assert im.dtype == torch.uint8 and im.dim() == 3 and im.is_contiguous()
    ptrs, hs, ws = _image_table(images_u8)
    check(_L().cddmsl_preprocess224_batch(ptrs, hs, ws, len(images_u8), ptr(out), Hp, Wp, RH, RW, top, left, size, Cp,
                                           m, s, DT[dtype], stream_ptr()), "cddmsl_preprocess224_batch")
    return out


@_timed("avgpool2_fwd")
def avgpool2_fwd(x):
    require_cuda(x)
    N, H, W, C = x.shape
    y = torch.empty((N, H // 2, W // 2, C), device=x.device, dtype=x.dtype)
    check(_L().cddmsl_avgpool2_fwd(ptr(x), ptr(y), N, H, W, C, _dt(x), stream_ptr()), "cddmsl_avgpool2_fwd")
    return y


@_timed("avgpool2_bwd")
def avgpool2_bwd(dy, in_shape, mask=None, add=None, emit8=None):
    require_cuda(dy, mask, add)
    N, H, W, C = in_shape
    assert dy.is_contiguous() and tuple(dy.shape) == (N, H // 2, W // 2, C)
    dx = torch.empty(in_shape, device=dy.device, dtype=dy.dtype)
    if emit8 is not None and dy.dtype == torch.bfloat16:
        y8 = torch.empty(in_shape, device=dy.device, dtype=torch.uint8)
        check(_L().cddmsl_avgpool2_bwd_q8(ptr(dy), ptr(mask), ptr(add), ptr(dx), N, H, W, C, ptr(y8), ptr(emit8[0]), ptr(emit8[1]), stream_ptr()),
              "cddmsl_avgpool2_bwd_q8")
        dx._fp8 = (y8, emit8[0].data_ptr())
        return dx
    check(_L().cddmsl_avgpool2_bwd(ptr(dy), ptr(mask), ptr(add), ptr(dx), N, H, W, C, _dt(dy), stream_ptr()), "cddmsl_avgpool2_bwd")
    return dx


@_timed("attn_tokens_fwd")
def attn_tokens_fwd(x, pos, tp=None):
    require_cuda(x, pos)
    K, P, C = x.shape
    tp = tp or P + 1
    assert pos.dtype == torch.float32 and tuple(pos.shape) == (P + 1, C) and x.is_contiguous() and pos.is_contiguous()
    tok = torch.empty((K, tp, C), device=x.device, dtype=x.dtype)
    check(_L().cddmsl_attn_tokens_fwd(ptr(x), ptr(pos), ptr(tok), K, P, tp, C, _dt(x), stream_ptr()), "cddmsl_attn_tokens_fwd")
    return tok


@_timed("attn_tokens_fwd")
def attn_tokens_fwd_mask(x, pos, tp=None):
    require_cuda(x, pos)
    K, P, C = x.shape
    tp = tp or P + 1
    assert pos.dtype == torch.float32 and tuple(pos.shape) == (P + 1, C) and x.is_contiguous() and pos.is_contiguous() and P <= 64
    tok = torch.empty((K, tp, C), device=x.device, dtype=x.dtype)
    mbits = torch.empty((K, C), device=x.device, dtype=torch.int64)
    check(_L().cddmsl_attn_tokens_fwd_mask(ptr(x), ptr(pos), ptr(tok), ptr(mbits), K, P, tp, C, _dt(x), stream_ptr()), "cddmsl_attn_tokens_fwd_mask")
    return tok, mbits


def rpn_losses(logits, deltas, pos, neg, midx, gt, gt_off, anchors, weights, inv_norm, gout=None):
    require_cuda(logits, deltas, pos, neg, midx, gt, gt_off, anchors)
    for t in (logits, deltas, gt, anchors):
        assert t.dtype == torch.float32 and t.is_contiguous()
    for t in (pos, neg, midx, gt_off):
        assert t.dtype == torch.int64 and t.is_contiguous()
    A = anchors.shape[0]
    assert deltas.numel() == 4 * logits.numel() and midx.numel() == logits.numel()
    args = (ptr(logits), ptr(deltas), ptr(pos), pos.numel(), ptr(neg), neg.numel(), ptr(midx), ptr(gt), ptr(gt_off), ptr(anchors), A,
            *[float(w) for w in weights], float(inv_norm))
    if gout is None:
        out = torch.empty(2, device=logits.device, dtype=torch.float32)
# ... 428 lines not shown

def cosine_logits_bwd(ds, x, wn, inv, temperature, dx=None):
    require_cuda(ds, x, wn, inv, dx)
    R, D = x.shape
    ds = ds.contiguous()
    assert x.dtype == wn.dtype == inv.dtype == ds.dtype == torch.float32 and x.is_contiguous() and wn.is_contiguous() and inv.is_contiguous()
    assert wn.dim() == 2 and wn.shape[1] == D and tuple(ds.shape) == (R, wn.shape[0] + 1) and inv.numel() == R
    acc = dx is not None
    if dx is None:
        dx = torch.empty_like(x)
    assert dx.dtype == torch.float32 and dx.is_contiguous() and dx.shape == x.shape
    check(_L().cddmsl_cosine_logits_bwd(ptr(ds), ptr(x), ptr(wn), ptr(inv), ptr(dx), R, D, wn.shape[0], temperature, int(acc),
                                         stream_ptr()), "cddmsl_cosine_logits_bwd")
    return dx


def contrastive_fwd(S):
    require_cuda(S)
    n = S.shape[0]
    assert S.dtype == torch.float32 and S.shape == (n, n) and S.is_contiguous()
    rl = torch.empty(n, device=S.device, dtype=torch.float32)
    cl = torch.empty(n, device=S.device, dtype=torch.float32)
    loss = torch.empty(1, device=S.device, dtype=torch.float32)
    check(_L().cddmsl_contrastive_fwd(ptr(S), ptr(rl), ptr(cl), ptr(loss), n, n, stream_ptr()), "cddmsl_contrastive_fwd")
    return loss, rl, cl


def contrastive_bwd(S, rl, cl, gloss):
    require_cuda(S, rl, cl, gloss)
    n = S.shape[0]
    assert S.dtype == rl.dtype == cl.dtype == torch.float32 and tuple(S.shape) == (n, n) and S.is_contiguous()
    assert rl.is_contiguous() and cl.is_contiguous() and rl.numel() == n and cl.numel() == n and gloss.numel() == 1
    dS = torch.empty_like(S)
    check(_L().cddmsl_contrastive_bwd(ptr(S), ptr(rl), ptr(cl), ptr(gloss.reshape(1).float().contiguous()), ptr(dS), n, n, stream_ptr()),
          "cddmsl_contrastive_bwd")
    return dS


@_timed("layernorm")
def layernorm_fwd(x, gamma, beta, out_dtype, eps=1e-5):
    require_cuda(x, gamma, beta)
    R, D = x.shape
    assert x.dtype == gamma.dtype == beta.dtype == torch.float32 and x.is_contiguous() and gamma.is_contiguous() and beta.is_contiguous()
    assert gamma.numel() == D and beta.numel() == D
    y = torch.empty((R, D), device=x.device, dtype=out_dtype)
    mean = torch.empty(R, device=x.device, dtype=torch.float32)
    rstd = torch.empty(R, device=x.device, dtype=torch.float32)
    check(_L().cddmsl_layernorm_fwd(ptr(x), ptr(gamma), ptr(beta), ptr(y), ptr(mean), ptr(rstd), R, D, eps, DT[out_dtype], stream_ptr()),
          "cddmsl_layernorm_fwd")
    return y, mean, rstd


@_timed("layernorm")
def layernorm_bwd(dy, x, gamma, mean, rstd, accumulate_into=None):
    require_cuda(dy, x, gamma, mean, rstd, accumulate_into)
    R, D = x.shape
    dy = dy.contiguous()
    assert x.dtype == gamma.dtype == mean.dtype == rstd.dtype == torch.float32 and x.is_contiguous() and gamma.is_contiguous()
    assert mean.is_contiguous() and rstd.is_contiguous() and gamma.numel() == D and mean.numel() == R and rstd.numel() == R and dy.shape == x.shape
    if accumulate_into is None:
        dx, acc = torch.empty_like(x), 0
    else:
        assert accumulate_into.dtype == torch.float32 and accumulate_into.is_contiguous() and accumulate_into.shape == x.shape
        dx, acc = accumulate_into, 1
    check(_L().cddmsl_layernorm_bwd(ptr(dy), ptr(x), ptr(gamma), ptr(mean), ptr(rstd), ptr(dx), R, D, acc, _dt(dy), stream_ptr()),
          "cddmsl_layernorm_bwd")
    return dx


def _attn_views(q, kv, t, heads):
    assert q.dim() == 2 and kv.dim() == 2 and q.is_contiguous() and kv.is_contiguous() and q.dtype == kv.dtype == torch.bfloat16
    R, d = q.shape
    assert kv.shape == (R, 2 * d) and R % t == 0 and d % heads == 0
    return R // t, d, d // heads


@_timed("attn_small")
def attn_small_fwd(q, kv, t, heads, scale):
    require_cuda(q, kv)
    n, d, dh = _attn_views(q, kv, t, heads)
    o = torch.empty_like(q)
    vptr = c_void_p(kv.data_ptr() + d * 2)
    check(_L().cddmsl_attn_small_fwd(ptr(q), ptr(kv), vptr, ptr(o), n, t, heads, dh, d, 2 * d, 2 * d, d, float(scale), 0, stream_ptr()),
          "cddmsl_attn_small_fwd")
    return o


@_timed("attn_last")
def attn_last_fwd(q, kv, t, heads, scale):
    require_cuda(q, kv)
    n, d = q.shape
    assert q.dtype == kv.dtype == torch.bfloat16 and q.is_contiguous() and kv.is_contiguous() and tuple(kv.shape) == (n * t, 2 * d)
    o = torch.empty((n, d), device=q.device, dtype=q.dtype)
    p = torch.empty((n, heads, t), device=q.device, dtype=torch.float32)
    check(_L().cddmsl_attn_last_fwd(ptr(q), ptr(kv), ptr(o), ptr(p), n, t, heads, d // heads, d, 2 * d, d, d, float(scale), 0, stream_ptr()),
          "cddmsl_attn_last_fwd")
    return o, p


@_timed("attn_last")
def attn_last_bwd(q, kv, do, p, t, heads, scale):
    require_cuda(q, kv, do, p)
    n, d = q.shape
    do = do.contiguous()
    assert do.shape == (n, d) and do.dtype == q.dtype and p.is_contiguous()
    dq, dkv = torch.empty_like(q), torch.empty_like(kv)
    check(_L().cddmsl_attn_last_bwd(ptr(q), ptr(kv), ptr(do), ptr(p), ptr(dq), ptr(dkv), n, t, heads, d // heads, d, 2 * d, d, d, float(scale), 0,
                                    stream_ptr()), "cddmsl_attn_last_bwd")
    return dq, dkv


@_timed("attn_small")
def attn_small_fwd_qkv(qkv, t, heads, scale):
    require_cuda(qkv)
    assert qkv.dim() == 2 and qkv.is_contiguous() and qkv.dtype == torch.bfloat16 and qkv.shape[1] % 3 == 0 and qkv.shape[0] % t == 0
    R, d = qkv.shape[0], qkv.shape[1] // 3
    o = torch.empty((R, d), device=qkv.device, dtype=qkv.dtype)
# ... 283 lines not shown
```

cddmsl_amd/layers.py:

```python
import os
import weakref

import torch

from . import hip

_STEP = [0]


def bump_weight_version():
    _STEP[0] += 1


_LOAD_GEN = [0]


def note_weights_loaded(*_):
    _LOAD_GEN[0] += 1
    _STEP[0] += 1


def load_generation():
    return _LOAD_GEN[0]

# ... 230 lines not shown
    key = (-1 if pw.frozen else _STEP[0], wd.data_ptr(), pw.param._version, _LOAD_GEN[0])
    c = getattr(pw, "_fp8d", None)
    if c is None or c[0] != key:
        amax = wd.abs().amax().float().clamp_min(1e-20).view(1)
        pw._fp8d = c = (key, hip.quantize_fp8(wd, hip.FP8_MAX / amax), amax / hip.FP8_MAX)
    return c[1], c[2]


def fp8_slot_of(owner, name):
    sl = getattr(owner, name, None)
    dev = (owner.param if hasattr(owner, "param") else owner.w[0]).device
    if sl is None or sl.scale.device != dev:
        sl = FP8_SCALES.slot(dev)
        setattr(owner, name, sl)
    return sl


def dgrad_auto(g, pw, fp8=False, slot=None, emit8=None, **kw):
    T = g.dtype
    _, wd = pw.get(T, True)
    if fp8 and T == torch.bfloat16 and slot is not None and not kw.get("residual_pooled", False):
        Cout_d, KH, KW, Cin_d = wd.shape
        pad = kw.get("pad", 0)
        N, H, W, _ = g.shape
        M = N * (H + 2 * pad - KH + 1) * (W + 2 * pad - KW + 1)
        if hip.conv_fwd_fp8_ok(M, Cin_d, Cout_d, KH, KW, pad):
            g8 = fp8_copy(g, slot)
            wd8, d_w = fp8_weight_d(pw, wd)
            return hip.conv_fwd_fp8(g8, wd8, (slot.deq * d_w).expand(Cout_d).contiguous(), None, kw.get("residual"), False, kw.get("relu_mask"),
                                    pad, emit8=emit8)
    if emit8 is not None:
        Cout_d, KH, KW, Cin_d = wd.shape
        N, H, W, _ = g.shape
        pad = kw.get("pad", 0)
        M = N * (H + 2 * pad - KH + 1) * (W + 2 * pad - KW + 1)
        if not (T == torch.bfloat16 and hip.conv_emit8_ok(M, Cout_d, KH, KW, (Cin_d * 2 // 16) % 8 == 0) and not kw.get("residual_pooled", False)):
            emit8 = None
    return hip.conv_fwd(g, wd, emit8=emit8, **kw)


def _fp8_dgrad_wanted(pw, g_shape, pad, fp8):
    if not fp8:
        return False
    Cout, KH, KW, Cin = _ohwi(pw.param).shape
    N, H, W, _ = g_shape
    M = N * (H + 2 * pad - KH + 1) * (W + 2 * pad - KW + 1)
    return hip.conv_fwd_fp8_ok(M, Cout, Cin, KH, KW, pad)


def cat_prepared(weights, dtype):
    return torch.cat([hip.weight_prep(_ohwi(w.detach()), None, dtype, True, False)[0] for w in weights], dim=0)


class ConvFn(torch.autograd.Function):

    @staticmethod
    def forward(ctx, x, anchor, pw, bias, stride, pad, relu, out_f32, train_w, residual=None, fp8=False):
        y = conv_fwd_auto(x, pw, None, None if bias is None else bias.detach(), fp8, residual=None if residual is None else residual.detach(),
                          relu=relu, stride=stride, pad=pad, out_f32=out_f32)
        ctx.pw, ctx.bias, ctx.cfg = pw, bias, (stride, pad, relu, out_f32, train_w)
        ctx.fp8 = bool(fp8)
        ctx.save_for_backward(x, y if relu else None, _fp8_made_for(x, pw) if fp8 else None)
        return y

    @staticmethod
    def backward(ctx, dy):
        x, y, x8 = ctx.saved_tensors
        stride, pad, relu, out_f32, train_w = ctx.cfg
        f8 = ctx.fp8 and x8 is not None and stride == 1
        g_slot = fp8_slot_of(ctx.pw, "_fp8_g") if f8 else None
        T = x.dtype
        dy_in = dy
        dy = dy.contiguous()
        if relu:
            dy = hip.relu_bwd(dy, y if y.dtype == T else y.to(T))
        elif dy.dtype != T:
            dy = dy.to(T)
        w = ctx.pw.param
        if train_w:
            if f8:
                wgrad_auto(x, dy, ctx.pw, None, pad, _ohwi(_grad_buf(w)), True, x8, g_slot, min_m=65536)
            else:
                hip.conv_wgrad(x, dy, _ohwi(w).shape, None, stride=stride, pad=pad, out=_ohwi(_grad_buf(w)))
            if ctx.bias is not None:
                hip.colsum(dy.view(-1, dy.shape[-1]), out=_grad_buf(ctx.bias))
        dx = None
        if ctx.needs_input_grad[0]:
            assert stride == 1, "input gradient of a strided conv is not on the hot path"
            _, wd = ctx.pw.get(T, need_dgrad=True)
            KH = _ohwi(w).shape[1]
            Kd, rows = dy.shape[-1], dy.numel() // dy.shape[-1]
            if KH == 1 and _ohwi(w).shape[2] == 1 and pad == 0 and rows <= 1024 and Kd >= 8192 and Kd % (16 * 64) == 0:
                S, N = 16, x.shape[-1]
                part = torch.empty(S, rows, N, device=dy.device, dtype=torch.float32)
                hip.gemm_nt_batched(dy, wd, part, rows, N, Kd // S, Kd, Kd, N, S, Kd // S, Kd // S, rows * N)
                dx = part.sum(0).to(T).view(x.shape)
            elif f8:
                dx = dgrad_auto(dy, ctx.pw, True, g_slot, pad=KH - 1 - pad)
            else:
                dx = hip.conv_fwd(dy, wd, stride=1, pad=KH - 1 - pad)
        return dx, None, None, None, None, None, None, None, None, (dy_in if ctx.needs_input_grad[9] else None), None


class FrozenMlpFn(torch.autograd.Function):

    @staticmethod
    def forward(ctx, x, pw1, b1, pw2, b2, residual):
        T = x.dtype
        w1, _ = pw1.get(T, need_dgrad=False)
        w2, _ = pw2.get(T, need_dgrad=False)
        M, K = x.shape
        h = hip.conv_fwd(x.view(1, 1, M, K), w1, None, b1.detach(), relu=True)
        y = hip.conv_fwd(h, w2, None, b2.detach(), residual.detach().view(1, 1, M, -1), out_f32=True)
        ctx.pw = (pw1, pw2)
        ctx.save_for_backward(h)
        return y.view(M, -1)

    @staticmethod
    def backward(ctx, dy):
        (h,) = ctx.saved_tensors
        T = h.dtype
        M = h.shape[2]
        g = dy.contiguous()
        if g.dtype != T:
            g = g.to(T)
        _, w2d = ctx.pw[1].get(T, need_dgrad=True)
        _, w1d = ctx.pw[0].get(T, need_dgrad=True)
        dh = hip.conv_fwd(g.view(1, 1, M, -1), w2d, relu_mask=h)
        dx = hip.conv_fwd(dh, w1d).view(M, -1) if ctx.needs_input_grad[0] else None
        return dx, None, None, None, None, (dy if ctx.needs_input_grad[5] else None)


def frozen_mlp(x2d, pw1, b1, pw2, b2, residual):
    return FrozenMlpFn.apply(x2d.contiguous(), pw1, b1, pw2, b2, residual.contiguous())


def conv(x, pw, bias=None, stride=1, pad=0, relu=False, out_f32=False, train_w=True, residual=None, fp8=False):
    anchor = pw.param if train_w else None
    assert residual is None or not relu
    return ConvFn.apply(x, anchor, pw, bias, stride, pad, relu, out_f32, train_w, residual, fp8)


def linear(x2d, pw, bias=None, relu=False, out_f32=False, train_w=True, residual=None):
    M, K = x2d.shape
    y = conv(x2d.contiguous().view(1, 1, M, K), pw, bias, 1, 0, relu, out_f32, train_w,
             None if residual is None else residual.contiguous().view(1, 1, M, -1))
    return y.view(M, -1)


class FusedHeadsFn(torch.autograd.Function):

    @staticmethod
    def forward(ctx, x, anchor, heads, out_f32):
        T = x.dtype
        K = heads[0][0].shape[1] if heads[0][0].dim() == 2 else heads[0][0].shape[1]
        ws = [w.detach().reshape(w.shape[0], -1) for w, _ in heads]
        n = sum(w.shape[0] for w in ws)
        npad = (n + 7) // 8 * 8
        wcat = torch.zeros(npad, 1, 1, ws[0].shape[1], device=x.device, dtype=torch.float32)
        wcat[:n, 0, 0] = torch.cat(ws, dim=0)
        bcat = torch.zeros(npad, device=x.device, dtype=torch.float32)
        bcat[:n] = torch.cat([b.detach() for _, b in heads])
        wf, wd = hip.weight_prep(wcat, None, T, True, True)
        y = hip.conv_fwd(x, wf, None, bcat, out_f32=out_f32)
        ctx.heads, ctx.wd, ctx.npad = heads, wd, npad
        ctx.save_for_backward(x)
        return y

    @staticmethod
    def backward(ctx, dy):
        (x,) = ctx.saved_tensors
        T = x.dtype
        dy = dy.contiguous()
        if dy.dtype != T:
            dy = dy.to(T)
        K = x.shape[-1]
        dw = hip.conv_wgrad(x, dy, (ctx.npad, 1, 1, K))
        db = hip.colsum(dy.view(-1, ctx.npad))
        off = 0
        for w, b in ctx.heads:
            n = w.shape[0]
            _grad_buf(w).view(n, -1).add_(dw[off:off + n].view(n, -1)) if w.dim() == 2 else \
                _ohwi(_grad_buf(w)).add_(dw[off:off + n])
            _grad_buf(b).add_(db[off:off + n])
            off += n
        dx = hip.conv_fwd(dy, ctx.wd) if ctx.needs_input_grad[0] else None
        return dx, None, None, None


def fused_heads(x, heads, out_f32=True):
    return FusedHeadsFn.apply(x, heads[0][0], heads, out_f32)


class BlockParams:

    def __init__(self, w1, w2, w3, wd, bn1, bn2, bn3, bnd, stride, frozen, fp8=False):
        self.stride, self.frozen, self.fp8 = stride, frozen, fp8
        self.bn = (bn1, bn2, bn3, bnd)
        self.w = (w1, w2, w3, wd)
        self.pw = tuple(None if w is None else PreparedWeight(w, b[0], frozen) for w, b in zip(self.w, self.bn))


def _block_forward(x, bp, save, px_given=None, next_pw=None, out_spec=None):
    (s1, b1), (s2, b2), (s3, b3), bnd = bp.bn
    pool = bp.stride > 1
    f8 = bp.fp8
    o1_shape = (x.shape[0], x.shape[1], x.shape[2], _ohwi(bp.w[0]).shape[0])
    o1 = conv_fwd_auto(x, bp.pw[0], s1, b1, f8, emit8=fp8_emit_for(bp.pw[1], o1_shape, 1, f8), relu=True)
    x8 = _fp8_made_for(x, bp.pw[0]) if f8 and save else None
    M2 = x.shape[0] * x.shape[1] * x.shape[2]
    e8o2 = fp8_act_slot(bp.pw[2]).emit() if save and not pool and _fp8_wgrad1x1_wanted(bp.pw[2], M2, f8) else None
    o2 = conv_fwd_auto(o1, bp.pw[1], s2, b2, f8, emit8=e8o2, relu=True, pad=1)
    o2_8 = _fp8_made_for(o2, bp.pw[2]) if e8o2 is not None else None
    p2 = hip.avgpool2_fwd(o2) if pool else o2
    if pool and px_given is not None and tuple(px_given.shape) == (x.shape[0], x.shape[1] // 2, x.shape[2] // 2, x.shape[3]):
        px = px_given
    else:
        px = hip.avgpool2_fwd(x) if pool else x
    if bp.pw[3] is not None:
        idn = conv_fwd_auto(px, bp.pw[3], bnd[0], bnd[1], f8)
    else:
        idn = x
    out_shape = (p2.shape[0], p2.shape[1], p2.shape[2], _ohwi(bp.w[2]).shape[0])
    out = conv_fwd_auto(p2, bp.pw[2], s3, b3, f8, emit8=fp8_emit_for(next_pw, out_shape, 0, f8), residual=idn, relu=True, out_spec=out_spec)
    return out, ((o1, o2, p2 if pool else None, px if pool else None, (x8, _fp8_made_for(o1, bp.pw[1]) if f8 else None, o2_8)) if save else None)


def _block_backward(gs, x, o1, o2, p2, px, bp, need_dx, mask_x, prev_bp=None, c8=(None, None, None)):
    T = x.dtype
    (s1, _), (s2, _), (s3, _), bnd = bp.bn
    pool = bp.stride > 1
    f8 = bp.fp8 and T == torch.bfloat16
    w1p, w2p, w3p, wdp = bp.w
    shp = lambda w: _ohwi(w).shape
    gs_slot = fp8_slot_of(bp, "_fp8_gs") if f8 else None
    d2_slot = fp8_slot_of(bp.pw[1], "_fp8_g") if f8 else None
    x8, o1_8, o2_8 = c8
    M2 = o2.shape[0] * o2.shape[1] * o2.shape[2]
    if o2_8 is not None and not pool:
        wgrad_auto(o2, gs, bp.pw[2], s3, 0, _ohwi(_grad_buf(w3p)), f8, o2_8, gs_slot, taps_only=False)
    else:
        hip.conv_wgrad(p2 if pool else o2, gs, shp(w3p), s3, out=_ohwi(_grad_buf(w3p)))
    d1_slot = fp8_slot_of(bp.pw[0], "_fp8_g") if f8 and x8 is not None and _fp8_wgrad1x1_wanted(bp.pw[0], M2, f8) else None
    if pool:
        dp2 = dgrad_auto(gs, bp.pw[2], f8, gs_slot)
        dpre2 = hip.avgpool2_bwd(dp2, tuple(o2.shape), mask=o2, emit8=d2_slot.emit() if f8 and _fp8_dgrad_wanted(bp.pw[1], o2.shape, 1, f8) else None)
    else:
        e8 = d2_slot.emit() if f8 and _fp8_dgrad_wanted(bp.pw[1], o2.shape, 1, f8) else None
        dpre2 = dgrad_auto(gs, bp.pw[2], f8, gs_slot, emit8=e8, relu_mask=o2)
    dpre1 = dgrad_auto(dpre2, bp.pw[1], f8, d2_slot, pad=1, relu_mask=o1, emit8=d1_slot.emit() if d1_slot is not None else None)
    wgrad_auto(o1, dpre2, bp.pw[1], s2, 1, _ohwi(_grad_buf(w2p)), f8, o1_8, d2_slot)
    if d1_slot is not None:
        wgrad_auto(x, dpre1, bp.pw[0], s1, 0, _ohwi(_grad_buf(w1p)), f8, x8, d1_slot, taps_only=False)
    else:
        hip.conv_wgrad(x, dpre1, shp(w1p), s1, out=_ohwi(_grad_buf(w1p)))
    if wdp is not None:
        hip.conv_wgrad(px if pool else x, gs, shp(wdp), bnd[0], out=_ohwi(_grad_buf(wdp)))
    if not need_dx:
        return None
    pooled = False
    if wdp is not None:
        dxb = dgrad_auto(gs, bp.pw[3], f8, gs_slot)
        if pool:
            pooled = x.shape[1] % 2 == 0 and x.shape[2] % 2 == 0 and hip.pooled_residual_ok(dxb)
            if not pooled:
                dxb = hip.avgpool2_bwd(dxb, tuple(x.shape))
    else:
        dxb = gs
    e8 = None
    if f8 and prev_bp is not None and prev_bp.fp8 and not pooled and _fp8_dgrad_wanted(prev_bp.pw[2], x.shape, 0, True):
        e8 = fp8_slot_of(prev_bp, "_fp8_gs").emit()
    return dgrad_auto(dpre1, bp.pw[0], False, None, emit8=e8, residual=dxb, relu_mask=x if mask_x else None, residual_pooled=pooled)


class ResStageFn(torch.autograd.Function):
    @staticmethod
    def forward(ctx, x, anchor, blocks, out_grad_premasked=False, px0=None, out_spec=None):
        ctx.out_grad_premasked = out_grad_premasked
        saved, o1_8s = [x], []
        cur = x
        for bi, bp in enumerate(blocks):
            cur, mids = _block_forward(cur, bp, True, px0 if bi == 0 else None, blocks[bi + 1].pw[0] if bi + 1 < len(blocks) else None,
                                       out_spec if bi + 1 == len(blocks) else None)
            saved += [mids[0], mids[1], mids[2], mids[3], cur]
            o1_8s += list(mids[4])
        ctx.blocks = blocks
        ctx.save_for_backward(*saved, *o1_8s)
        return cur

    @staticmethod
    def backward(ctx, g):
        blocks = ctx.blocks
        saved, o1_8s = ctx.saved_tensors[:-3 * len(blocks)], ctx.saved_tensors[-3 * len(blocks):]
        need_dx = ctx.needs_input_grad[0]
        gs = g.contiguous() if ctx.out_grad_premasked else hip.relu_bwd(g.contiguous(), saved[-1])
        for i in range(len(blocks) - 1, -1, -1):
            x, o1, o2, p2, px = saved[5 * i: 5 * i + 5]
            gs = _block_backward(gs, x, o1, o2, p2, px, blocks[i], need_dx or i > 0, mask_x=i > 0, prev_bp=blocks[i - 1] if i > 0 else None,
                                 c8=tuple(o1_8s[3 * i: 3 * i + 3]))
        return gs, None, None, None, None, None


def _fused_stage_ok(x, blocks, out_spec):
    if os.environ.get("CDDMSL_FUSED_BOTTLENECK", "1") == "0" or out_spec is not None:
        return False
    if not (x.is_cuda and x.dtype == torch.bfloat16 and x.dim() == 4 and x.is_contiguous()):
        return False
    cin = x.shape[3]
    for bi, bp in enumerate(blocks):
        if bp.fp8 or bp.stride != 1 or any(v is None for b in bp.bn[:3] for v in b):
            return False
        if tuple(_ohwi(bp.w[0]).shape) != (64, 1, 1, cin) or tuple(_ohwi(bp.w[1]).shape) != (64, 3, 3, 64) or tuple(_ohwi(bp.w[2]).shape) != (256, 1, 1, 64):
            return False
        if bp.w[3] is not None:
            if bi > 0 or cin != 64 or tuple(_ohwi(bp.w[3]).shape) != (256, 1, 1, 64) or any(v is None for v in bp.bn[3]):
                return False
        elif cin != 256:
            return False
        cin = 256
    return bool(blocks) and bool(hip._L().cddmsl_bottleneck64_ok(x.shape[0], x.shape[1], x.shape[2], 0))


def _fused_stage_forward(x, blocks):
    T = x.dtype
    wf = lambda pw: pw.get(T, need_dgrad=False)[0]
    o1 = conv_fwd_auto(x, blocks[0].pw[0], blocks[0].bn[0][0], blocks[0].bn[0][1], False, relu=True)
    cur = x
    for bi, bp in enumerate(blocks):
        nxt = blocks[bi + 1] if bi + 1 < len(blocks) else None
        kw = dict(x0=cur, wd=wf(bp.pw[3]), bnd=bp.bn[3]) if bp.pw[3] is not None else dict(residual=cur)
        if nxt is not None:
            kw.update(w1n=wf(nxt.pw[0]), bn1n=nxt.bn[0])
        cur, o1 = hip.bottleneck64_fwd(o1, wf(bp.pw[1]), bp.bn[1], wf(bp.pw[2]), bp.bn[2], **kw)
    return cur


def res_stage(x, blocks, frozen, out_grad_premasked=False, out_spec=None):
    px0 = getattr(x, "_pooled2", None)
    if frozen or not torch.is_grad_enabled():
        if _fused_stage_ok(x, blocks, out_spec):
            return _fused_stage_forward(x, blocks)
        cur = x
        for bi, bp in enumerate(blocks):
            cur, _ = _block_forward(cur, bp, False, px0 if bi == 0 else None, blocks[bi + 1].pw[0] if bi + 1 < len(blocks) else None,
                                    out_spec if bi + 1 == len(blocks) else None)
        return cur
    return ResStageFn.apply(x, blocks[0].w[0], blocks, out_grad_premasked, px0, out_spec)


class StackHalvesFn(torch.autograd.Function):

    @staticmethod
    def forward(ctx, a, b, full):
        n = a.shape[0]
        assert a.data_ptr() == full.data_ptr() and b.data_ptr() == full[n:].data_ptr() and full.shape[0] == 2 * n and a.shape == b.shape
        ctx.n = n
        return full.view(full.shape)

    @staticmethod
    def backward(ctx, g):
        return g[:ctx.n], g[ctx.n:], None


def stack_halves(a, b, full):
    return StackHalvesFn.apply(a, b, full)


def res_stage_attnpool(x, blocks, frozen, ap):
    fuse = not frozen and torch.is_grad_enabled()
    y = res_stage(x, blocks, frozen, out_grad_premasked=fuse)
    return AttnPoolFn.apply(y, None if ap.frozen else ap.q_w, ap, fuse)


def roi_downsample_on_map(K, out_size, N, H, W):
    if os.environ.get("CDDMSL_ROI_COMMUTE", "1") == "0":
        return False
    v = os.environ.get("CDDMSL_ROI_COMMUTE_DOWN", "")
    if v in ("0", "1"):
        return v == "1"
    return K * (out_size // 2) ** 2 > N * H * W


def _roi_block0_forward(feat, rois, bp, out_size, scale, sr, extra, next_pw=None, on_map=None):
    T = feat.dtype
    (s1, b1), (s2, b2), (s3, b3), bnd = bp.bn
    w1, _ = bp.pw[0].get(T, False)
    f8 = bp.fp8
    K, E = rois.shape[0], (0 if extra is None else extra.shape[0])
    N, H, W, _ = feat.shape
    z = hip.conv_fwd(feat, w1)
    o1_shape = (K + E, out_size, out_size, z.shape[-1])
    e8 = fp8_emit_for(bp.pw[1], o1_shape, 1, f8) if E == 0 else None
    o1 = hip.roi_align_forward_affine(z, rois, out_size, out_size, scale, sr, True, s1, b1, relu=True, extra_rows=E, emit8=e8)
    del z
    if on_map is None:
        on_map = roi_downsample_on_map(K, out_size, N, H, W)
    if on_map:
        wd, _ = bp.pw[3].get(T, False)
        zd = hip.conv_fwd(feat, wd)
        idn = hip.roi_align_forward_affine(zd, rois, out_size, out_size, scale, sr, True, bnd[0], bnd[1], pooled_only=True, extra_rows=E)
        del zd
        px = None
        if E:
            px = hip.avgpool2_fwd(extra)
            idn[K:].copy_(hip.conv_fwd(px, wd, bnd[0], bnd[1]))
    else:
        px = hip.roi_align_forward_affine(feat, rois, out_size, out_size, scale, sr, True, pooled_only=True, extra_rows=E)
        idn = None
    if E:
        o1[K:].copy_(hip.conv_fwd(extra, w1, s1, b1, relu=True))
        if idn is None:
            px[K:].copy_(hip.avgpool2_fwd(extra))
    o2 = conv_fwd_auto(o1, bp.pw[1], s2, b2, f8, relu=True, pad=1)
    p2 = hip.avgpool2_fwd(o2)
    if idn is None:
        idn = conv_fwd_auto(px, bp.pw[3], bnd[0], bnd[1], f8)
    out_shape = (p2.shape[0], p2.shape[1], p2.shape[2], _ohwi(bp.w[2]).shape[0])
    out = conv_fwd_auto(p2, bp.pw[2], s3, b3, f8, emit8=fp8_emit_for(next_pw, out_shape, 0, f8), residual=idn, relu=True)
    return o1, o2, p2, px, out, (_fp8_made_for(o1, bp.pw[1]) if f8 else None)


class RoIStageFn(torch.autograd.Function):

    @staticmethod
    def forward(ctx, feat, anchor, rois, roi_start, blocks, out_size, scale, sr, out_grad_premasked, extra):
        feat = feat.contiguous()
        nxt = lambda i: blocks[i + 1].pw[0] if i + 1 < len(blocks) else None
        on_map = roi_downsample_on_map(rois.shape[0], out_size, feat.shape[0], feat.shape[1], feat.shape[2])
        o1, o2, p2, px, cur, o1_8 = _roi_block0_forward(feat, rois, blocks[0], out_size, scale, sr, extra, nxt(0), on_map)
        saved, o1_8s = [feat, rois, roi_start, extra, o1, o2, p2, px, cur], [None, o1_8, None]
        for bi, bp in enumerate(blocks[1:], start=1):
            cur, mids = _block_forward(cur, bp, True, None, nxt(bi))
            saved += [mids[0], mids[1], mids[2], mids[3], cur]
            o1_8s += list(mids[4])
        ctx.blocks, ctx.meta = blocks, (out_size, scale, sr, out_grad_premasked, on_map)
        ctx.save_for_backward(*saved, *o1_8s)
        return cur

    @staticmethod
    def backward(ctx, g):
        blocks = ctx.blocks
        saved, o1_8s = ctx.saved_tensors[:-3 * len(blocks)], ctx.saved_tensors[-3 * len(blocks):]
        out_size, scale, sr, premasked, on_map = ctx.meta
        feat, rois, roi_start, extra = saved[:4]
        st = saved[4:]
        gs = g.contiguous() if premasked else hip.relu_bwd(g.contiguous(), st[-1])
        for i in range(len(blocks) - 1, 0, -1):
            o1, o2, p2, px = st[5 * i: 5 * i + 4]
            gs = _block_backward(gs, st[5 * i - 1], o1, o2, p2, px, blocks[i], True, mask_x=True, prev_bp=blocks[i - 1], c8=tuple(o1_8s[3 * i: 3 * i + 3]))
        bp = blocks[0]
        o1, o2, p2, px = st[0:4]
        T = o1.dtype
        (s1, _), (s2, _), (s3, _), bnd = bp.bn
        w1p, w2p, w3p, wdp = bp.w
        shp = lambda w: _ohwi(w).shape
        K, E = rois.shape[0], (0 if extra is None else extra.shape[0])
        f8 = bp.fp8 and T == torch.bfloat16
        gs_slot = fp8_slot_of(bp, "_fp8_gs") if f8 else None
        d2_slot = fp8_slot_of(bp.pw[1], "_fp8_g") if f8 else None
        hip.conv_wgrad(p2, gs, shp(w3p), s3, out=_ohwi(_grad_buf(w3p)))
        e8 = d2_slot.emit() if f8 and _fp8_dgrad_wanted(bp.pw[1], o2.shape, 1, f8) else None
        dpre2 = hip.avgpool2_bwd(dgrad_auto(gs, bp.pw[2], f8, gs_slot), tuple(o2.shape), mask=o2, emit8=e8)
        dpre1 = dgrad_auto(dpre2, bp.pw[1], f8, d2_slot, pad=1, relu_mask=o1)
        wgrad_auto(o1, dpre2, bp.pw[1], s2, 1, _ohwi(_grad_buf(w2p)), f8, o1_8s[1], d2_slot)
        N, H, W, C = feat.shape
        _, w1d = bp.pw[0].get(T, True)
        dfeat = dextra = dzd = wdd = None
        if on_map:
            _, wdd = bp.pw[3].get(T, True)
            dzd = hip.roi_align_backward(gs[:K], rois, roi_start, (N, H, W, gs.shape[-1]), scale, sr, True, pooled=True)
            hip.conv_wgrad(feat, dzd, shp(wdp), bnd[0], out=_ohwi(_grad_buf(wdp)))
            if E:
                hip.conv_wgrad(px, gs[K:], shp(wdp), bnd[0], out=_ohwi(_grad_buf(wdp)))
        else:
            hip.conv_wgrad(px, gs, shp(wdp), bnd[0], out=_ohwi(_grad_buf(wdp)))
            dxb = dgrad_auto(gs, bp.pw[3], f8, gs_slot)
        dz = hip.roi_align_backward(dpre1[:K], rois, roi_start, (N, H, W, dpre1.shape[-1]), scale, sr, True)
        hip.conv_wgrad(feat, dz, shp(w1p), s1, out=_ohwi(_grad_buf(w1p)))
        if E:
            hip.conv_wgrad(extra, dpre1[K:], shp(w1p), s1, out=_ohwi(_grad_buf(w1p)))
            if ctx.needs_input_grad[9]:
                dxe = hip.conv_fwd(gs[K:], wdd) if on_map else dxb[K:].contiguous()
                dextra = hip.conv_fwd(dpre1[K:], w1d, residual=hip.avgpool2_bwd(dxe, tuple(extra.shape)))
        if ctx.needs_input_grad[0]:
            r = hip.conv_fwd(dzd, wdd) if on_map else hip.roi_align_backward(dxb[:K], rois, roi_start, (N, H, W, C), scale, sr, True, pooled=True)
            dfeat = hip.conv_fwd(dz, w1d, residual=r)
        return dfeat, None, None, None, None, None, None, None, None, dextra


def roi_stage_supported(blocks):
    bp = blocks[0]
    return bp.stride == 2 and bp.w[3] is not None and tuple(bp.w[0].shape[2:]) == (1, 1) and tuple(bp.w[3].shape[2:]) == (1, 1)


def roi_stage(feat, rois, roi_start, blocks, frozen, out_size, scale, sr, extra=None, out_grad_premasked=False):
    assert rois.dim() == 2 and rois.size(1) == 5 and out_size % 2 == 0
    assert extra is None or tuple(extra.shape[1:]) == (out_size, out_size, feat.shape[3])
    if frozen or not torch.is_grad_enabled():
        nxt = lambda i: blocks[i + 1].pw[0] if i + 1 < len(blocks) else None
        cur = _roi_block0_forward(feat.contiguous(), rois, blocks[0], out_size, scale, sr, extra, nxt(0))[4]
        for bi, bp in enumerate(blocks[1:], start=1):
            cur, _ = _block_forward(cur, bp, False, None, nxt(bi))
        return cur
    return RoIStageFn.apply(feat, blocks[0].w[0], rois, roi_start, blocks, out_size, scale, sr, out_grad_premasked, extra)


def roi_stage_attnpool(feat, rois, roi_start, blocks, frozen, ap, out_size, scale, sr, extra=None):
    fuse = not frozen and torch.is_grad_enabled()
    y = roi_stage(feat, rois, roi_start, blocks, frozen, out_size, scale, sr, extra, out_grad_premasked=fuse)
    return AttnPoolFn.apply(y, None if ap.frozen else ap.q_w, ap, fuse)


class RoIAlignFn(torch.autograd.Function):
    @staticmethod
    def forward(ctx, x, rois, roi_start, out_size, scale, sampling_ratio, aligned, with_pooled=False, extra=None):
# ... 180 lines not shown

class ContrastiveFn(torch.autograd.Function):

    @staticmethod
    def forward(ctx, a, b):
        an, ia = hip.l2norm_fwd(a.contiguous(), 0.0)
        bn, ib = hip.l2norm_fwd(b.contiguous(), 0.0)
        S = hip.linear_fwd(an, bn)
        loss, rl, cl = hip.contrastive_fwd(S)
        ctx.save_for_backward(an, ia, bn, ib, S, rl, cl)
        return loss.view(())

    @staticmethod
    def backward(ctx, g):
        an, ia, bn, ib, S, rl, cl = ctx.saved_tensors
        dS = hip.contrastive_bwd(S, rl, cl, g)
        n = dS.shape[0]
        pad = (-n) % 4
        P = (lambda t: torch.nn.functional.pad(t, (0, pad))) if pad else (lambda t: t)
        dan = hip.linear_fwd(P(dS).contiguous(), P(bn.t()).contiguous())
        dbn = hip.linear_fwd(P(dS.t()).contiguous(), P(an.t()).contiguous())
        return hip.l2norm_bwd(dan, an, ia), hip.l2norm_bwd(dbn, bn, ib)


def contrastive_loss(a, b):
    return ContrastiveFn.apply(a, b)


class LayerNormFn(torch.autograd.Function):

    @staticmethod
    def forward(ctx, x, gamma, beta, out_dtype):
        y, mean, rstd = hip.layernorm_fwd(x.contiguous(), gamma, beta, out_dtype)
        ctx.save_for_backward(x, gamma, mean, rstd)
        return y

    @staticmethod
    def backward(ctx, dy):
        x, gamma, mean, rstd = ctx.saved_tensors
        return hip.layernorm_bwd(dy, x.contiguous(), gamma, mean, rstd), None, None, None


def layer_norm(x2d, gamma, beta, out_dtype):
    return LayerNormFn.apply(x2d, gamma.detach(), beta.detach(), out_dtype)


class LayerNormSkipFn(torch.autograd.Function):

    @staticmethod
    def forward(ctx, x, gamma, beta, out_dtype):
        x = x.contiguous()
        y, mean, rstd = hip.layernorm_fwd(x, gamma, beta, out_dtype)
        ctx.save_for_backward(x, gamma, mean, rstd)
        return y, x.view_as(x)

    @staticmethod
    def backward(ctx, dy, dskip):
        x, gamma, mean, rstd = ctx.saved_tensors
        if dskip is None:
            return hip.layernorm_bwd(dy, x, gamma, mean, rstd), None, None, None
        acc = dskip.contiguous()
        if dy is None:
            return acc, None, None, None
        return hip.layernorm_bwd(dy, x, gamma, mean, rstd, accumulate_into=acc), None, None, None


def layer_norm_skip(x2d, gamma, beta, out_dtype):
    return LayerNormSkipFn.apply(x2d, gamma.detach(), beta.detach(), out_dtype)


class FocalCEFn(torch.autograd.Function):

    @staticmethod
    def forward(ctx, logits, target, gamma, bg_class, bg_weight):
        logits = logits.contiguous()
        row, probs = hip.focal_ce_fwd(logits, target, gamma, bg_class, bg_weight)
        ctx.save_for_backward(logits, target, probs)
        ctx.meta = (gamma, bg_class, bg_weight)
        return row.mean()

    @staticmethod
    def backward(ctx, g):
        logits, target, probs = ctx.saved_tensors
        gamma, bg_class, bg_weight = ctx.meta
        return hip.focal_ce_bwd(logits, target, probs, g / logits.shape[0], gamma, bg_class, bg_weight), None, None, None, None


def focal_cross_entropy(logits, target, gamma, bg_class, bg_weight):
    return FocalCEFn.apply(logits, target, float(gamma or 0.0), int(bg_class), float(1.0 if bg_weight is None else bg_weight))


class RpnLossesFn(torch.autograd.Function):

    @staticmethod
    def forward(ctx, logits, deltas, pos, neg, midx, gt, gt_off, anchors, weights, inv_norm):
        logits, deltas = logits.contiguous(), deltas.contiguous()
        ctx.save_for_backward(logits, deltas, pos, neg, midx, gt, gt_off, anchors)
        ctx.cfg = (weights, inv_norm)
        return hip.rpn_losses(logits, deltas, pos, neg, midx, gt, gt_off, anchors, weights, inv_norm)

    @staticmethod
    def backward(ctx, g):
        logits, deltas, pos, neg, midx, gt, gt_off, anchors = ctx.saved_tensors
        dl, dd = hip.rpn_losses(logits, deltas, pos, neg, midx, gt, gt_off, anchors, ctx.cfg[0], ctx.cfg[1], gout=g)
        return dl, dd, None, None, None, None, None, None, None, None


def rpn_losses(logits, deltas, pos, neg, midx, gt, gt_off, anchors, weights, inv_norm):
    return RpnLossesFn.apply(logits, deltas, pos, neg, midx, gt, gt_off, anchors, tuple(weights), float(inv_norm))


class BoxL1Fn(torch.autograd.Function):

    @staticmethod
    def forward(ctx, deltas, fg, cls, src, tgt, weights, inv_norm):
        deltas = deltas.contiguous()
# ... 124 lines not shown
```

cddmsl_amd/modeling/backbone.py:

```python
from collections import OrderedDict

import torch
from torch import nn

from .. import hip, layers
from ..registry import BACKBONE_REGISTRY
from ..structures import ShapeSpec


def to_nhwc(x):
    v = x.permute(0, 2, 3, 1)
    return v if v.is_contiguous() else v.contiguous()


def to_nchw(x):
    return x.permute(0, 3, 1, 2)


class Conv2dW(nn.Module):

    def __init__(self, cin, cout, k):
        super().__init__()
        w = torch.empty(cout, cin, k, k).contiguous(memory_format=torch.channels_last)
        self.weight = nn.Parameter(w)


class FrozenBatchNorm2d(nn.Module):

    def __init__(self, num_features, eps=1e-5):
        super().__init__()
        self.num_features, self.eps = num_features, eps
        self.register_buffer("weight", torch.ones(num_features))
        self.register_buffer("bias", torch.zeros(num_features))
        self.register_buffer("running_mean", torch.zeros(num_features))
        self.register_buffer("running_var", torch.ones(num_features) - eps)
        self._aff = None

    def affine(self):
        if self._aff is None or self._aff[0].device != self.weight.device:
            scale = self.weight * (self.running_var + self.eps).rsqrt()
            bias = self.bias - self.running_mean * scale
            self._aff = (scale.float().contiguous(), bias.float().contiguous())
        return self._aff

    def _load_from_state_dict(self, *a, **k):
        self._aff = None
        layers.note_weights_loaded()
        return super()._load_from_state_dict(*a, **k)


class Bottleneck(nn.Module):
    expansion = 4
# ... 80 lines not shown
        self._out_features = list(out_features) if out_features else []
        ch = {"stem": width, "res2": width * 4, "res3": width * 8, "res4": width * 16, "res5": width * 32}
        st = {"stem": 4, "res2": 4, "res3": 8, "res4": 16, "res5": 32}
        self._out_feature_channels = {k: ch[k] for k in ch if k != "res5" or "res5" in self._out_features}
        self._out_feature_strides = {k: st[k] for k in self._out_feature_channels}
        self._stem_w = None
        self.freeze(freeze_at)

    def _make_layer(self, planes, blocks, stride=1):
        ls = [Bottleneck(self._inplanes, planes, stride)]
        self._inplanes = planes * 4
        for _ in range(1, blocks):
            ls.append(Bottleneck(self._inplanes, planes))
        return ResStage(*ls)

    @property
    def size_divisibility(self):
        return 0

    def output_shape(self):
        return {n: ShapeSpec(channels=self._out_feature_channels[n], stride=self._out_feature_strides[n])
                for n in self._out_features}

    def freeze(self, freeze_at=0):
        assert freeze_at >= 1, "the HIP stem path has no backward: MODEL.BACKBONE.FREEZE_AT must be >= 1"
        self.freeze_at = freeze_at
        for m in (self.conv1, self.conv2, self.conv3):
            m.weight.requires_grad = False
        for idx, stage in enumerate([self.layer1, self.layer2, self.layer3, self.layer4], start=2):
            if freeze_at >= idx:
                for blk in stage:
                    blk.frozen = True
                    for p in blk.parameters():
                        p.requires_grad = False
        return self

    def _stem_weights(self, T, cp):
        dev = self.conv1.weight.device
        key = (T, cp, dev, layers.load_generation(), self.conv1.weight._version, self.conv2.weight._version, self.conv3.weight._version)
        if self._stem_w is None or self._stem_w[0] != key:
            w1 = torch.zeros(self.conv1.weight.shape[0], 3, 3, cp, device=dev)
            w1[..., :3] = self.conv1.weight.detach().permute(0, 2, 3, 1)
            ws = [hip.weight_prep(w1, None, T, True, False)[0],
                  hip.weight_prep(layers._ohwi(self.conv2.weight.detach()), None, T, True, False)[0],
                  hip.weight_prep(layers._ohwi(self.conv3.weight.detach()), None, T, True, False)[0]]
            self._stem_w = (key, ws)
        return self._stem_w[1]

    def stem_nhwc(self, x):
        w1, w2, w3 = self._stem_weights(x.dtype, x.shape[-1])
        (s1, b1), (s2, b2), (s3, b3) = self.bn1.affine(), self.bn2.affine(), self.bn3.affine()
        x = hip.conv_fwd(x, w1, s1, b1, relu=True, stride=2, pad=1)
        x = hip.conv_fwd(x, w2, s2, b2, relu=True, pad=1)
        x = hip.conv_fwd(x, w3, s3, b3, relu=True, pad=1)
        return hip.avgpool2_fwd(x)

    def forward_nhwc(self, x, want_res5=None, res4_spec=None):
        with torch.no_grad():
            x = self.stem_nhwc(x)
        x = self.layer1.forward_nhwc(x)
        x = self.layer2.forward_nhwc(x)
        res4 = self.layer3.forward_nhwc(x, out_spec=res4_spec)
        out = {"res4": res4}
        if "res5" in self._out_features and want_res5 is not False:
            out["res5"] = self.layer4.forward_nhwc(res4)
        return out

    def forward(self, x, want_res5=None):
        assert x.dim() == 4, f"ResNet takes an input of shape (N, C, H, W). Got {x.shape} instead!"
        T = self.compute_dtype
        cp = 8 if T == torch.bfloat16 else 4
        xin = torch.zeros(x.shape[0], x.shape[2], x.shape[3], cp, device=x.device, dtype=T)
        xin[..., :3] = x.permute(0, 2, 3, 1)
        return {k: to_nchw(v) for k, v in self.forward_nhwc(xin, want_res5).items()}


@BACKBONE_REGISTRY.register()
def build_clip_resnet_backbone(cfg, input_shape=None):
    depth = cfg.MODEL.RESNETS.DEPTH
    blocks = {50: [3, 4, 6, 3], 101: [3, 4, 23, 3], 200: [4, 6, 10, 6]}[depth]
    width = {50: 64, 101: 64, 200: 80}[depth]
    embed_dim = {50: 1024, 101: 512, 200: 640}[depth]
    res = {50: 224, 101: 224, 200: 288}[depth]
    mode = cfg.MODEL.get("COMPUTE_DTYPE", "bf16")
    dt = {"bf16": torch.bfloat16, "f32": torch.float32, "fp8": torch.bfloat16}[mode]
    net = ModifiedResNet(blocks, embed_dim, width * 32 // 64, res, width, cfg.MODEL.RESNETS.OUT_FEATURES,
                         cfg.MODEL.BACKBONE.FREEZE_AT, depth, False, True, dt)
    if mode == "fp8":
        for m in net.modules():
            if isinstance(m, Bottleneck):
                m.fp8 = True
    return net


def build_backbone(cfg, input_shape=None):
    if input_shape is None:
        input_shape = ShapeSpec(channels=len(cfg.MODEL.PIXEL_MEAN))
    return BACKBONE_REGISTRY.get(cfg.MODEL.BACKBONE.NAME)(cfg, input_shape)
```

include/cddmsl_hip.h:

```cpp
#ifndef CDDMSL_HIP_H
#define CDDMSL_HIP_H
#include <stddef.h>

#ifdef __cplusplus
extern "C" {
#endif

int cddmsl_abi_version(void);

int cddmsl_conv_fwd(const void* x, const void* w, void* y, const float* scale, const float* bias, const void* residual,
                    const void* relu_mask, int Nimg, int Hi, int Wi, int Cin, int Cout, int KH, int KW, int stride, int pad,
                    int pool, int ldy, int ldr, int ldm, int relu, int out_f32, int dtype, void* stream);
int cddmsl_bottleneck64_ok(int Nimg, int H, int W, int dtype);
int cddmsl_bottleneck64_fwd(const void* o1, const void* w2, const float* s2, const float* b2, const void* w3, const float* s3,
                            const float* b3, const void* residual, const void* x0, const void* wd, const float* sd,
                            const float* bd, const void* w1n, const float* s1n, const float* b1n, void* out, void* o1n,
                            int Nimg, int H, int W, int dtype, void* stream);
int cddmsl_set_workspace(void* ptr, long bytes);
int cddmsl_conv_wgrad(const void* x, const void* dy, float* dw, const float* scale, int Nimg, int Hi, int Wi, int Cin,
                      int Cout, int KH, int KW, int stride, int pad, int pool, int ldd, int dtype, void* stream);
int cddmsl_gemm_nt_batched(const void* a, const void* w, void* c, const float* bias, int M, int N, int K, int lda, int ldb, int ldc,
                           int batch, long sa, long sw, long sc, int out_f32, int dtype, void* stream);
int cddmsl_gemm_tn_batched(const void* a, const void* b, void* out, int M, int N, int K, int lda, int ldb, int ldo, int batch, long sa,
                           long sb, long so, int mode, int dtype, void* stream);
int cddmsl_last_kernel(void);
int cddmsl_plan_only(int on);
int cddmsl_weight_prep(const float* w, const float* scale, void* w_fwd, void* w_dgrad, int Cout, int KH, int KW, int Cin,
                       int dtype, void* stream);
int cddmsl_weight_prep_multi(const long long* table, int count, int dtype, void* stream);

int cddmsl_quantize_fp8(const void* x, void* y, const float* scale, float* amax, long numel, int src_dtype, void* stream);
int cddmsl_conv_fwd_fp8(const void* x, const void* w, void* y, const float* scale, const float* bias, const void* residual,
                        const void* relu_mask, int Nimg, int Hi, int Wi, int Cin, int Cout, int KH, int KW, int pad, int relu,
                        int out_f32, void* y8, const float* q8, float* amax8, void* stream);
int cddmsl_conv_fwd_q8(const void* x, const void* w, void* y, const float* scale, const float* bias, const void* residual,
                       const void* relu_mask, int Nimg, int Hi, int Wi, int Cin, int Cout, int KH, int KW, int stride, int pad,
                       int relu, void* y8, const float* q8, float* amax8, void* stream);
int cddmsl_fp8_dot_nt(const void* a, const void* b, float* c, const float* alpha, int R, int N, int K, int ldc, void* stream);
int cddmsl_conv_wgrad_fp8_ok(int Cin, int Cout, int KH, int KW, int pad, int ldd);
int cddmsl_conv_wgrad_fp8(const void* x8, const void* dy8, float* dw, const float* scale, int Nimg, int Hi, int Wi, int Cin, int Cout,
                          int KH, int KW, int pad, int ldd, void* stream);

int cddmsl_roi_align_forward(const void* x, const float* rois, void* y, void* y_pooled, int* dbg_grid, int N, int C, int H, int W,
                             int K, int ph, int pw, float spatial_scale, int sampling_ratio, int aligned, int dtype, void* stream);
int cddmsl_roi_align_backward(const void* dy, const float* rois, const int* roi_start, void* dx, float* ws_ay, float* ws_ax,
                              int* ws_fp, int N, int C, int H, int W, int K, int ph, int pw, float spatial_scale,
                              int sampling_ratio, int aligned, int dtype, void* stream);
int cddmsl_roi_align_forward_affine(const void* x, const float* rois, void* y, void* y_pooled, const float* scale,
                                    const float* bias, int relu, int N, int C, int H, int W, int K, int ph, int pw,
                                    float spatial_scale, int sampling_ratio, int aligned, int dtype, void* y8, const float* q8,
                                    float* amax8, void* stream);
int cddmsl_roi_align_backward_pooled(const void* dy, const float* rois, const int* roi_start, void* dx, float* ws_ay,
                                     float* ws_ax, int* ws_fp, int N, int C, int H, int W, int K, int ph, int pw,
                                     float spatial_scale, int sampling_ratio, int aligned, int dtype, void* stream);
int cddmsl_roi_align_nchw_anyorder(const void* input, const float* rois, void* output, int N, int C, int H, int W, int K, int ph, int pw,
                                   float spatial_scale, int sampling_ratio, int aligned, int dtype, void* temp, size_t* temp_bytes,
                                   void* stream);
int cddmsl_roi_align_backward_nchw_anyorder(const void* grad, const float* rois, void* grad_input, int N, int C, int H, int W, int K,
                                            int ph, int pw, float spatial_scale, int sampling_ratio, int aligned, int dtype, void* temp,
                                            size_t* temp_bytes, void* stream);

int cddmsl_anchors(const float* cell, float* out, int Hf, int Wf, int A, float stride, float offset, void* stream);
int cddmsl_sort_desc(const float* keys_in, float* keys_out, int* idx_scratch, int* order_out, const int* offsets, int N,
                     int total, void* temp, size_t* temp_bytes, void* stream);
int cddmsl_rpn_decode(const int* order, const float* deltas, const float* cell, const int* img_hw, float* boxes,
// ... 20 lines not shown
                           void* stream);
int cddmsl_attnpool_softmax_fwd(const float* S, float* p, void* pT, long K, int H, int P1, int TP, float scale, int dtype, void* stream);
int cddmsl_attnpool_softmax_bwd(const float* p, const float* dP, void* dsT, void* pds, long K, int H, int P1, int TP, float scale,
                                int dtype, void* stream);

int cddmsl_attn_small_fwd(const void* q, const void* k, const void* v, void* o, int nseq, int t, int heads, int dh, int ldq,
                          int ldk, int ldv, int ldo, float scale, int dtype, void* stream);
int cddmsl_attn_small_bwd(const void* q, const void* k, const void* v, const void* dout, void* dq, void* dk, void* dv, int nseq,
                          int t, int heads, int dh, int ldq, int ldk, int ldv, int ldo, float scale, int dtype, void* stream);
int cddmsl_attn_last_fwd(const void* q, const void* kv, void* o, float* p, int n, int t, int heads, int dh, int ldq, int ldkv, int voff,
                         int ldo, float scale, int dtype, void* stream);
int cddmsl_attn_last_bwd(const void* q, const void* kv, const void* dout, const float* p, void* dq, void* dkv, int n, int t, int heads,
                         int dh, int ldq, int ldkv, int voff, int ldo, float scale, int dtype, void* stream);

int cddmsl_text_embed(const long* ids, const void* tok, const float* pos, float* x, long rows, int t, int W, int vocab, int dtype,
                      void* stream);
int cddmsl_attn_causal_fwd(const void* qkv, void* o, int nseq, int t, int heads, int dh, int ldqkv, int ldo, float scale, int dtype,
                           void* stream);
int cddmsl_quick_gelu(void* x, long numel, int dtype, void* stream);
int cddmsl_text_pool(const float* x, const long* rows, const float* gamma, const float* beta, void* y, long R, int nout, int group,
                     int W, float eps, int dtype, void* stream);

int cddmsl_skinny_gemm_workspace(int M, int N, int K);
int cddmsl_skinny_gemm(const void* x, const void* w, const float* bias, const float* residual, void* y, float* ws, long ws_bytes, int M,
                       int N, int K, int epi, void* stream);
int cddmsl_lm_head_workspace(int M, int V);
int cddmsl_lm_head_argmax(const void* h, const void* wte, long* ids, int ld_ids, float* logits, void* ws, long ws_bytes, int M, int V,
                          int K, void* stream);
int cddmsl_decode_attn(const void* qkv, void* kc, void* vc, void* o, int nseq, int heads, int dh, int L, int Lmax, int ldqkv, float scale,
                       int dtype, void* stream);
int cddmsl_pos_embed(const long* ids, int ld_ids, const void* tab, const float* src, const float* wpe, float* x, long rows, int t, int pos0,
                     int W, int vocab, int npos, int dtype, void* stream);
int cddmsl_gelu_new(void* x, long numel, int dtype, void* stream);
int cddmsl_lm_head_topk_workspace(int M, int V);
int cddmsl_lm_head_topk(const void* h, const void* wte, float* vals, int* idx, float* logZ, float* logits, void* ws, long ws_bytes, int M,
                        int V, int K, int B, void* stream);
int cddmsl_beam_step(const float* vals, const int* idx, const float* logZ, const float* sum_in, const int* len_in,
                     const unsigned char* stop_in, const int* hist_in, const unsigned char* anc_in, float* sum_out, int* len_out,
                     unsigned char* stop_out, int* hist_out, unsigned char* anc_out, int* src, long* next_tok, int n, int B, int T, int step,
                     int stop_id, void* stream);
int cddmsl_decode_attn_beam(const void* qkv, const void* pk, const void* pv, void* gk, void* gv, const unsigned char* anc, void* o, int rows,
                            int B, int heads, int dh, int P, int L, int Tg, int ldanc, int ldqkv, float scale, int dtype, void* stream);

int cddmsl_l2norm_fwd(const float* x, float* y, float* inv, long R, int D, float eps, void* stream);
int cddmsl_l2norm_bwd(const float* dy, const float* y, const float* inv, float* dx, long R, int D, void* stream);
int cddmsl_cosine_logits_fwd(const float* x, const float* wn, float* scores, float* inv, long R, int D, int Kc,
                             float temperature, float eps, void* stream);
int cddmsl_cosine_logits_bwd(const float* ds, const float* x, const float* wn, const float* inv, float* dx, long R, int D,
                             int Kc, float temperature, int accumulate, void* stream);
int cddmsl_layernorm_fwd(const float* x, const float* gamma, const float* beta, void* y, float* mean, float* rstd, long R, int D,
                         float eps, int dtype, void* stream);
int cddmsl_layernorm_bwd(const void* dy, const float* x, const float* gamma, const float* mean, const float* rstd, float* dx,
                         long R, int D, int accumulate, int dtype, void* stream);
int cddmsl_focal_ce_fwd(const float* logits, const long* target, float* row_loss, float* probs, long R, int C, float gamma,
                        int bg_class, float bg_weight, void* stream);
int cddmsl_focal_ce_bwd(const float* logits, const long* target, const float* probs, const float* gscale, float* dlogits, long R,
                        int C, float gamma, int bg_class, float bg_weight, void* stream);
int cddmsl_contrastive_fwd(const float* S, float* rlse, float* clse, float* loss, int n, int ld, void* stream);
int cddmsl_contrastive_bwd(const float* S, const float* rlse, const float* clse, const float* gloss, float* dS, int n, int ld,
                           void* stream);
int cddmsl_rpn_losses(const float* logits, const float* deltas, const long* pos, int npos, const long* neg, int nneg, const long* midx,
                      const float* gt, const long* gt_off, const float* anchors, long A, float wx, float wy, float ww, float wh, float inv_norm,
                      float* out2, const float* gout2, float* dlogits, float* ddeltas, void* stream);
int cddmsl_box_l1(const float* deltas, int ld, const long* fg, int nfg, const long* cls, const float* src, const float* tgt, float wx, float wy,
                  float ww, float wh, float inv_norm, float* out1, const float* gout1, float* ddeltas, void* stream);

int cddmsl_preprocess(const unsigned char* img, void* out, int n, int h, int w, int Hp, int Wp, int Cp, const float* mean3,
                      const float* std3, int div255, int dtype, void* stream);
int cddmsl_preprocess224(const unsigned char* img, void* out, int n, int h, int w, int Hp, int Wp, int RH, int RW, int top,
                         int left, int S, int Cp, const float* mean3, const float* std3, int dtype, void* stream);
int cddmsl_preprocess_batch(const unsigned char* const* imgs, const int* hs, const int* ws, int N, void* out, int Hp, int Wp, int Cp,
                            const float* mean3, const float* std3, int div255, int dtype, void* stream);
int cddmsl_preprocess224_batch(const unsigned char* const* imgs, const int* hs, const int* ws, int N, void* out, int Hp, int Wp, int RH,
                               int RW, int top, int left, int S, int Cp, const float* mean3, const float* std3, int dtype, void* stream);
int cddmsl_avgpool2_fwd(const void* x, void* y, int N, int H, int W, int C, int dtype, void* stream);
int cddmsl_avgpool2_bwd(const void* dy, const void* mask, const void* add, void* dx, int N, int H, int W, int C, int dtype,
                        void* stream);
int cddmsl_avgpool2_bwd_q8(const void* dy, const void* mask, const void* add, void* dx, int N, int H, int W, int C, void* y8,
                           const float* q8, float* amax8, void* stream);
int cddmsl_maxpool3s2_fwd(const void* x, void* y, int N, int H, int W, int C, int dtype, void* stream);
int cddmsl_upsample_zero2(const void* t, const void* mask, const void* add, void* dx, int N, int H, int W, int C, int dtype,
                          void* stream);
int cddmsl_meanpool_fwd(const void* x, float* y, long K, int P, int C, int dtype, void* stream);
int cddmsl_meanpool_bwd(const float* dy, void* dx, long K, int P, int C, int dtype, void* stream);
int cddmsl_relu_bwd(const void* g, const void* y, void* dx, long numel, int g_f32, int dtype, void* stream);
int cddmsl_colsum(const void* x, float* out, long rows, int cols, int period, int dtype, void* stream);
int cddmsl_sgd_clip_step(float** params, const float** grads, float** moms, const long* sizes, int count, float* norm_ws,
                         float lr, float momentum, float wd, float clip, int first_step, void* stream);

int cddmsl_instance_boxes(const void* maps, int B, int H, int W, int dtype, int* records, int max_records, int* counts, void* ws,
                          size_t* ws_bytes, void* stream);

#ifdef __cplusplus
}
#endif
#endif
```

Baseline: 172.4.

## Fuse stem conv with avgpool, bitpack pool masks, emit bf16 layernorm grads

After: 174.5, median of 6. 1.01x the previous value.

```diff
diff --git a/cddmsl_amd/csrc/conv_fwd.hip b/cddmsl_amd/csrc/conv_fwd.hip
--- a/cddmsl_amd/csrc/conv_fwd.hip
+++ b/cddmsl_amd/csrc/conv_fwd.hip
@@ -479,8 +479,9 @@
   }
 }
 
-template <typename T, int CPP, int NT, int NTAP = 9>
+template <typename T, int CPP, int NT, int NTAP = 9, bool POOL = false>
 __global__ __launch_bounds__(256) void k_conv3x3_small(ConvArgs p) {
+  static_assert(!POOL || (Mma<T>::ES == 2 && NT == 2 && NTAP == 9 && CPP > 1), "pooled output: the bf16 3x3 instantiation with 64 output channels");
   constexpr int KC = NTAP * CPP, KS = (KC + 1) / 2;
   constexpr int PAD = NTAP == 9 ? 1 : 0;
   constexpr int ES = Mma<T>::ES;
@@ -507,20 +508,33 @@
 #pragma unroll
   for (int nt = 0; nt < NT; ++nt) { sc[nt] = p.scale ? p.scale[nt * 32 + r] : 1.f; bi[nt] = p.bias ? p.bias[nt * 32 + r] : 0.f; }
   const int wave = (blockIdx.x * blockDim.x + threadIdx.x) >> 6, nwaves = (gridDim.x * blockDim.x) >> 6;
-  const int ntiles = (p.M + 31) >> 5;
+  const int Hp = p.Ho >> 1, Wp = p.Wo >> 1, Mp = POOL ? p.Nimg * Hp * Wp : 0;
+  const int ntiles = POOL ? (Mp + 7) >> 3 : (p.M + 31) >> 5;
   const __amdgpu_buffer_rsrc_t rx = __builtin_amdgcn_make_buffer_rsrc((void*)(p.x - (long)(p.Wi + 1) * (CPP * 16)), 0, 0x7fffffff, 0x00020000);
-  const long ybytes = (long)p.M * p.ldy * ES, mbytes = (long)p.M * p.ldm * ES;
+  const long ybytes = (long)(POOL ? Mp : p.M) * p.ldy * ES, mbytes = (long)p.M * p.ldm * ES;
   const __amdgpu_buffer_rsrc_t ry = __builtin_amdgcn_make_buffer_rsrc((void*)p.y, 0, (int)(ybytes > 0x7fffffffL ? 0x7fffffffL : ybytes), 0x00020000);
   const __amdgpu_buffer_rsrc_t rm = __builtin_amdgcn_make_buffer_rsrc((void*)p.relu_mask, 0, p.relu_mask ? (int)(mbytes > 0x7fffffffL ? 0x7fffffffL : mbytes) : 0, 0x00020000);
   const float relu_floor = p.relu ? 0.f : -__builtin_inff();
   __shared__ __attribute__((aligned(16))) u32x4 ost[ES == 2 ? 4 * 32 * NT * 4 : 1];
   const bool ost_ok = !p.relu_mask && p.ldy == NT * 32 && (long)p.M * NT * 64 < 0x7fffffffL;
   for (int tile = wave; tile < ntiles; tile += nwaves) {
-    const int m = tile * 32 + r;
-    const bool vm = m < p.M;
-    const unsigned mm = vm ? m : 0;
-    const unsigned tq = fdiv(mm, p.dWo), ox = mm - tq * p.Wo;
-    const unsigned img = fdiv(tq, p.dHo), oy = tq - img * p.Ho;
+    bool vm;
+    unsigned ox, oy, img;
+    if (POOL) {
+      const int q = tile * 8 + (r >> 2);
+      vm = q < Mp;
+      const unsigned qq = vm ? q : 0;
+      const unsigned tq = fdiv(qq, p.dWp), pox = qq - tq * Wp;
+      img = fdiv(tq, p.dHp);
+      oy = 2 * (tq - img * Hp) + ((r >> 1) & 1); ox = 2 * pox + (r & 1);
+    } else {
+      const int m = tile * 32 + r;
+      vm = m < p.M;
+      const unsigned mm = vm ? m : 0;
+      const unsigned tq = fdiv(mm, p.dWo);
+      ox = mm - tq * p.Wo;
+      img = fdiv(tq, p.dHo); oy = tq - img * p.Ho;
+    }
     const int iy0 = (int)oy * p.stride - PAD, ix0 = (int)ox * p.stride - PAD;
     const unsigned lbase = (unsigned)((((int)img * p.Hi + iy0 + 1) * p.Wi + ix0 + 1) * (CPP * 16)) + (CPP > 1 ? hh * 16 : 0);
     unsigned bad = vm ? 0u : 0x1ffu;
@@ -563,6 +577,26 @@
         if (WLDS) Mma<T>::step(acc[nt], a[ks], wl[(nt * KS + ks) * 64 + wlane]);
         else Mma<T>::step(acc[nt], a[ks], bw[WLDS ? 0 : nt][WLDS ? 0 : ks]);
       }
+    if (POOL) {
+      char* ob = (char*)ost + (threadIdx.x >> 6) * (32 * NT * 64);
+#pragma unroll
+      for (int nt = 0; nt < NT; ++nt)
+#pragma unroll
+        for (int k = 0; k < 4; ++k) {
+          float a4[4];
+#pragma unroll
+          for (int j = 0; j < 4; ++j) {
+            float v = affine<T>(acc[nt][4 * k + j], sc[nt], bi[nt]);
+            asm("v_max_f32 %0, %1, %2" : "=v"(v) : "v"(v), "s"(relu_floor));
+            a4[j] = bf2f(f2bf(v));
+          }
+          *(unsigned short*)(ob + (2 * k + hh) * (NT * 64) + (nt * 32 + r) * 2) = f2bf(((a4[0] + a4[1]) + (a4[2] + a4[3])) * 0.25f);
+        }
+      static_assert(!POOL || NT == 2, "one 1 KiB store per pooled tile");
+      const u32x4 o = *(const u32x4*)(ob + lane * 16);
+      __builtin_amdgcn_raw_buffer_store_b128(o, ry, (unsigned)(lane * 16), tile * (8 * NT * 64), 0);
+      continue;
+    }
     if (ES == 2 && ost_ok) {
       char* ob = (char*)ost + (threadIdx.x >> 6) * (32 * NT * 64);
 #pragma unroll
@@ -608,6 +642,9 @@
   else if (a.cpp == 1) hipLaunchKernelGGL((k_conv3x3_small<T, 1, 2>), dim3(nb), dim3(256), 0, st, a);
   else if (a.cpp == 8) hipLaunchKernelGGL((k_conv3x3_small<T, 8, 2>), dim3(nb), dim3(256), 0, st, a);
   else if (a.Cout == 32) hipLaunchKernelGGL((k_conv3x3_small<T, 4, 1>), dim3(nb), dim3(256), 0, st, a);
+  else if (a.pool_out) {
+    if constexpr (sizeof(T) == 2) hipLaunchKernelGGL((k_conv3x3_small<T, 4, 2, 9, true>), dim3(nb), dim3(256), 0, st, a);
+  }
   else hipLaunchKernelGGL((k_conv3x3_small<T, 4, 2>), dim3(nb), dim3(256), 0, st, a);
 }
 
diff --git a/cddmsl_amd/csrc/elementwise.hip b/cddmsl_amd/csrc/elementwise.hip
--- a/cddmsl_amd/csrc/elementwise.hip
+++ b/cddmsl_amd/csrc/elementwise.hip
@@ -166,6 +166,50 @@
   }
 }
 
+__global__ void k_avgpool2_fwd_bits(const char* x, char* y, unsigned* bits, int N, int H, int W, int cch) {
+  using T = __bf16;
+  int Ho = H / 2, Wo = W / 2;
+  long total = (long)N * Ho * Wo * cch;
+  for (long i = (long)blockIdx.x * blockDim.x + threadIdx.x; i < total; i += (long)gridDim.x * blockDim.x) {
+    int c = i % cch; long q = i / cch;
+    int ox = q % Wo; q /= Wo;
+    int oy = q % Ho; int n = q / Ho;
+    const u32x4* b = (const u32x4*)x + (((long)n * H + 2 * oy) * W + 2 * ox) * cch + c;
+    float a0[8], a1[8], a2[8], a3[8], o[8];
+    Elt<T>::unpack(b[0], a0); Elt<T>::unpack(b[cch], a1);
+    Elt<T>::unpack(b[(long)W * cch], a2); Elt<T>::unpack(b[(long)W * cch + cch], a3);
+    unsigned m = 0u;
+#pragma unroll
+    for (int j = 0; j < 8; ++j) {
+      o[j] = ((a0[j] + a1[j]) + (a2[j] + a3[j])) * 0.25f;
+      m |= (a0[j] > 0.f ? 1u : 0u) << j | (a1[j] > 0.f ? 1u : 0u) << (8 + j) | (a2[j] > 0.f ? 1u : 0u) << (16 + j) | (a3[j] > 0.f ? 1u : 0u) << (24 + j);
+    }
+    ((u32x4*)y)[i] = Elt<T>::pack(o);
+    bits[i] = m;
+  }
+}
+__global__ void k_avgpool2_bwd_bits(const char* dy, const unsigned* bits, char* dx, int N, int H, int W, int cch) {
+  using T = __bf16;
+  int Ho = H / 2, Wo = W / 2;
+  long total = (long)N * H * W * cch;
+  for (long i = (long)blockIdx.x * blockDim.x + threadIdx.x; i < total; i += (long)gridDim.x * blockDim.x) {
+    int c = i % cch; long q = i / cch;
+    int xx = q % W; q /= W;
+    int yy = q % H; int n = q / H;
+    float g[8], o[8];
+    bool in = (yy >> 1) < Ho && (xx >> 1) < Wo;
+    unsigned m = 0u;
+    if (in) {
+      const long p = (((long)n * Ho + (yy >> 1)) * Wo + (xx >> 1)) * cch + c;
+      Elt<T>::unpack(((const u32x4*)dy)[p], g);
+      m = bits[p] >> (8 * ((yy & 1) * 2 + (xx & 1)));
+    }
+#pragma unroll
+    for (int j = 0; j < 8; ++j) o[j] = (in && ((m >> j) & 1u)) ? g[j] * 0.25f : 0.f;
+    ((u32x4*)dx)[i] = Elt<T>::pack(o);
+  }
+}
+
 __global__ __launch_bounds__(256) void k_avgpool2_bwd_q8(const char* dy, const char* mask, const char* add, char* dx, int N, int H, int W, int cch,
                                                          char* y8, const float* q8, unsigned* amax8) {
   using T = __bf16;
@@ -648,6 +692,23 @@
   return launch_status();
 }
 
+extern "C" int cddmsl_avgpool2_fwd_bits(const void* x, void* y, void* bits, int N, int H, int W, int C, int dtype, void* stream) {
+  if (dtype != 0 || C % 8 || H < 2 || W < 2 || !bits) return CDDMSL_ERR_ARG;
+  const int cch = C / 8;
+  const long total = (long)N * (H / 2) * (W / 2) * cch;
+  if (total == 0) return CDDMSL_OK;
+  hipLaunchKernelGGL(k_avgpool2_fwd_bits, dim3(gsz(total)), dim3(256), 0, (hipStream_t)stream, (const char*)x, (char*)y, (unsigned*)bits, N, H, W, cch);
+  return launch_status();
+}
+extern "C" int cddmsl_avgpool2_bwd_bits(const void* dy, const void* bits, void* dx, int N, int H, int W, int C, int dtype, void* stream) {
+  if (dtype != 0 || C % 8 || H < 2 || W < 2 || !bits) return CDDMSL_ERR_ARG;
+  const int cch = C / 8;
+  const long total = (long)N * H * W * cch;
+  if (total == 0) return CDDMSL_OK;
+  hipLaunchKernelGGL(k_avgpool2_bwd_bits, dim3(gsz(total)), dim3(256), 0, (hipStream_t)stream, (const char*)dy, (const unsigned*)bits, (char*)dx, N, H, W, cch);
+  return launch_status();
+}
+
 extern "C" int cddmsl_avgpool2_bwd_q8(const void* dy, const void* mask, const void* add, void* dx, int N, int H, int W, int C, void* y8,
                                       const float* q8, float* amax8, void* stream) {
   if ((C * 2) % 16 || !y8 || !q8 || !amax8) return CDDMSL_ERR_ARG;
diff --git a/cddmsl_amd/csrc/gemm_common.h b/cddmsl_amd/csrc/gemm_common.h
--- a/cddmsl_amd/csrc/gemm_common.h
+++ b/cddmsl_amd/csrc/gemm_common.h
@@ -53,6 +53,8 @@
   unsigned* amax8 = nullptr;
   float* partial = nullptr;
   int tile0 = 0, ksplits = 1, kper = 0, tile_limit = 0;
+  int pool_out = 0;
+  FastDiv dWp = {}, dHp = {};
   int nt_out = 1;
 #ifdef CDDMSL_TILE_STAMPS
   unsigned long long* tstamps = nullptr;
diff --git a/cddmsl_amd/csrc/gemm_conv.hip b/cddmsl_amd/csrc/gemm_conv.hip
--- a/cddmsl_amd/csrc/gemm_conv.hip
+++ b/cddmsl_amd/csrc/gemm_conv.hip
@@ -193,6 +193,21 @@
                       relu, out_f32, nullptr, nullptr, nullptr, stream);
 }
 
+extern "C" int cddmsl_conv3x3_pool_fwd(const void* x, const void* w, void* y, const float* scale, const float* bias, const void* relu_mask,
+                                       int Nimg, int Hi, int Wi, int Cin, int Cout, int stride, int dtype, void* stream) {
+  if (dtype != 0 || Cin != 32 || Cout != 64 || stride != 1 || relu_mask || !scale || !bias || Hi < 2 || Wi < 2) return CDDMSL_ERR_ARG;
+  ConvArgs a;
+  const int st = fill_conv(a, OP_BF16, x, w, y, scale, bias, nullptr, nullptr, Nimg, Hi, Wi, Cin, Cout, 3, 3, 1, 1, 0, Cout, 0, 0, 1, 0,
+                           nullptr, nullptr, nullptr);
+  if (st != CDDMSL_OK || a.M == 0) return st;
+  if ((long)Nimg * Hi * Wi * Cin * 2 >= 0x7ffff000L || (long)Nimg * (a.Ho / 2) * (a.Wo / 2) * Cout * 2 >= 0x7fffffffL) return CDDMSL_ERR_ARG;
+  a.pool_out = 1;
+  a.dWp = make_fastdiv((unsigned)(a.Wo / 2)); a.dHp = make_fastdiv((unsigned)(a.Ho / 2));
+  const Plan pl = plan_fwd(a, OP_BF16, 1);
+  if (pl.kernel != 8) return CDDMSL_ERR_ARG;
+  return run_fwd(a, OP_BF16, pl, stream);
+}
+
 extern "C" int cddmsl_conv_fwd_q8(const void* x, const void* w, void* y, const float* scale, const float* bias,
                                   const void* residual, const void* relu_mask, int Nimg, int Hi, int Wi, int Cin,
                                   int Cout, int KH, int KW, int stride, int pad, int relu, void* y8, const float* q8, float* amax8,
diff --git a/cddmsl_amd/csrc/losses.hip b/cddmsl_amd/csrc/losses.hip
--- a/cddmsl_amd/csrc/losses.hip
+++ b/cddmsl_amd/csrc/losses.hip
@@ -224,10 +224,11 @@
   }
   if (lane == 0) { mean[r] = mu; rstd[r] = rs; }
 }
-template <typename T, int NSEG>
+template <typename T, int NSEG, bool EMIT = false>
 __global__ __launch_bounds__(256) void k_layernorm_bwd_v(const void* __restrict__ dy, const float* __restrict__ x,
                                                          const float* __restrict__ gamma, const float* __restrict__ mean,
-                                                         const float* __restrict__ rstd, float* dx, long R, int accumulate) {
+                                                         const float* __restrict__ rstd, float* dx, long R, int accumulate,
+                                                         void* dxb = nullptr) {
   constexpr int D = NSEG * 256;
   const long r = (long)blockIdx.x * 4 + (threadIdx.x >> 6);
   const int lane = threadIdx.x & 63;
@@ -257,6 +258,7 @@
     v.z = rs * (g[s].z - sg - xh[s].z * sgx); v.w = rs * (g[s].w - sg - xh[s].w * sgx);
     if (accumulate) { v.x = o[s].x + v.x; v.y = o[s].y + v.y; v.z = o[s].z + v.z; v.w = o[s].w + v.w; }
     dxr[s * 64 + lane] = v;
+    if (EMIT) st4((__bf16*)nullptr, dxb, r * (D / 4) + s * 64 + lane, v);
   }
 }
 template <typename T> bool layernorm_fwd_v(const float* x, const float* gamma, const float* beta, void* y, float* mean, float* rstd,
@@ -271,8 +273,17 @@
   return false;
 }
 template <typename T> bool layernorm_bwd_v(const void* dy, const float* x, const float* gamma, const float* mean, const float* rstd,
-                                           float* dx, long R, int D, int accumulate, hipStream_t st) {
+                                           float* dx, long R, int D, int accumulate, hipStream_t st, void* dxb = nullptr) {
   const dim3 grid((unsigned)((R + 3) / 4)), blk(256);
+  if (dxb) {
+    switch (D) {
+      case 256: k_layernorm_bwd_v<T, 1, true><<<grid, blk, 0, st>>>(dy, x, gamma, mean, rstd, dx, R, accumulate, dxb); return true;
+      case 512: k_layernorm_bwd_v<T, 2, true><<<grid, blk, 0, st>>>(dy, x, gamma, mean, rstd, dx, R, accumulate, dxb); return true;
+      case 768: k_layernorm_bwd_v<T, 3, true><<<grid, blk, 0, st>>>(dy, x, gamma, mean, rstd, dx, R, accumulate, dxb); return true;
+      case 1024: k_layernorm_bwd_v<T, 4, true><<<grid, blk, 0, st>>>(dy, x, gamma, mean, rstd, dx, R, accumulate, dxb); return true;
+    }
+    return false;
+  }
   switch (D) {
     case 256: k_layernorm_bwd_v<T, 1><<<grid, blk, 0, st>>>(dy, x, gamma, mean, rstd, dx, R, accumulate); return true;
     case 512: k_layernorm_bwd_v<T, 2><<<grid, blk, 0, st>>>(dy, x, gamma, mean, rstd, dx, R, accumulate); return true;
@@ -389,6 +400,19 @@
   if (dtype == 0) k_layernorm_bwd<__bf16><<<grid, dim3(256), 0, (hipStream_t)stream>>>(dy, x, gamma, mean, rstd, dx, R, D, accumulate);
   else k_layernorm_bwd<float><<<grid, dim3(256), 0, (hipStream_t)stream>>>(dy, x, gamma, mean, rstd, dx, R, D, accumulate);
   return launch_status();
+}
+extern "C" int cddmsl_layernorm_bwd_emit(const void* dy, const float* x, const float* gamma, const float* mean, const float* rstd,
+                                         float* dx, void* dx_bf16, long R, int D, int accumulate, int dtype, int* emitted, void* stream) {
+  if (R < 0 || D <= 0 || (dtype != 0 && dtype != 1) || !dx_bf16 || !emitted) return CDDMSL_ERR_ARG;
+  *emitted = 0;
+  if (R == 0) return CDDMSL_OK;
+  if (aligned16(dy, x, gamma, dx, dx_bf16) &&
+      (dtype == 0 ? layernorm_bwd_v<__bf16>(dy, x, gamma, mean, rstd, dx, R, D, accumulate, (hipStream_t)stream, dx_bf16)
+                  : layernorm_bwd_v<float>(dy, x, gamma, mean, rstd, dx, R, D, accumulate, (hipStream_t)stream, dx_bf16))) {
+    *emitted = 1;
+    return launch_status();
+  }
+  return cddmsl_layernorm_bwd(dy, x, gamma, mean, rstd, dx, R, D, accumulate, dtype, stream);
 }
 extern "C" int cddmsl_focal_ce_fwd(const float* logits, const long* target, float* row_loss, float* probs, long R, int C,
                                    float gamma, int bg_class, float bg_weight, void* stream) {
diff --git a/cddmsl_amd/hip.py b/cddmsl_amd/hip.py
--- a/cddmsl_amd/hip.py
+++ b/cddmsl_amd/hip.py
@@ -36,6 +36,9 @@
         L.cddmsl_avgpool2_fwd.argtypes = [vp, vp] + [ci] * 5 + [vp]
         L.cddmsl_avgpool2_bwd.argtypes = [vp] * 4 + [ci] * 5 + [vp]
         L.cddmsl_avgpool2_bwd_q8.argtypes = [vp] * 4 + [ci] * 4 + [vp] * 4
+        L.cddmsl_avgpool2_fwd_bits.argtypes = [vp] * 3 + [ci] * 5 + [vp]
+        L.cddmsl_avgpool2_bwd_bits.argtypes = [vp] * 3 + [ci] * 5 + [vp]
+        L.cddmsl_conv3x3_pool_fwd.argtypes = [vp] * 6 + [ci] * 7 + [vp]
         L.cddmsl_attn_tokens_fwd.argtypes = [vp] * 3 + [ci] * 5 + [vp]
         L.cddmsl_attn_tokens_bwd.argtypes = [vp] * 4 + [ci] * 5 + [vp]
         L.cddmsl_attnpool_softmax_fwd.argtypes = [vp] * 3 + [c_long, ci, ci, ci, cf, ci, vp]
@@ -70,6 +73,7 @@
         L.cddmsl_cosine_logits_bwd.argtypes = [vp] * 5 + [c_long, ci, ci, cf, ci, vp]
         L.cddmsl_layernorm_fwd.argtypes = [vp] * 6 + [c_long, ci, cf, ci, vp]
         L.cddmsl_layernorm_bwd.argtypes = [vp] * 6 + [c_long, ci, ci, ci, vp]
+        L.cddmsl_layernorm_bwd_emit.argtypes = [vp] * 7 + [c_long, ci, ci, ci, ctypes.POINTER(ci), vp]
         L.cddmsl_focal_ce_fwd.argtypes = [vp] * 4 + [c_long, ci, cf, ci, cf, vp]
         L.cddmsl_focal_ce_bwd.argtypes = [vp] * 5 + [c_long, ci, cf, ci, cf, vp]
         L.cddmsl_attn_small_fwd.argtypes = [vp] * 4 + [ci] * 8 + [cf, ci, vp]
@@ -260,6 +264,28 @@
     return y
 
 
+def conv3x3_pool_fwd(x, w, scale, bias, relu_mask=None, stride=1):
+    require_cuda(x, w, scale, bias, relu_mask)
+    assert x.dim() == 4 and w.dim() == 4 and x.is_contiguous() and w.is_contiguous() and x.dtype == w.dtype
+    N, H, W, Cin = x.shape
+    Cout, KH, KW, Cin2 = w.shape
+    assert (KH, KW, Cin2) == (3, 3, Cin), (x.shape, w.shape)
+    for v in (scale, bias):
+        assert v is not None and v.dtype == torch.float32 and v.numel() == Cout and v.is_contiguous()
+    assert relu_mask is None or (relu_mask.dtype == x.dtype and relu_mask.is_contiguous())
+    y = torch.empty((N, H // 2, W // 2, Cout), device=x.device, dtype=x.dtype)
+
+    def launch():
+        return _L().cddmsl_conv3x3_pool_fwd(ptr(x), ptr(w), ptr(y), ptr(scale), ptr(bias), ptr(relu_mask), N, H, W, Cin, Cout, stride,
+                                            _dt(x), stream_ptr())
+    e0 = PROFILE.begin(plan=launch) if PROFILE.on else None
+    check(launch(), "cddmsl_conv3x3_pool_fwd")
+    Mc = N * (H // 2) * (W // 2) * 4
+    PROFILE.end(e0, "k_conv3x3_small", 2.0 * Mc * Cout * 9 * Cin, (Mc, Cout, 9 * Cin, 3, 2, 1),
+                nbytes=float(x.numel() * x.element_size() + w.numel() * w.element_size() + y.numel() * y.element_size()))
+    return y
+
+
 def bottleneck64_ok(o1, w2, w3, wd=None, w1n=None):
     if not (o1.is_cuda and o1.dtype == torch.bfloat16 and o1.dim() == 4 and o1.is_contiguous() and o1.shape[3] == 64):
         return False
@@ -508,6 +534,28 @@
     y = torch.empty((N, H // 2, W // 2, C), device=x.device, dtype=x.dtype)
     check(_L().cddmsl_avgpool2_fwd(ptr(x), ptr(y), N, H, W, C, _dt(x), stream_ptr()), "cddmsl_avgpool2_fwd")
     return y
+
+
+@_timed("avgpool2_fwd")
+def avgpool2_fwd_bits(x):
+    require_cuda(x)
+    assert x.dtype == torch.bfloat16 and x.is_contiguous()
+    N, H, W, C = x.shape
+    y = torch.empty((N, H // 2, W // 2, C), device=x.device, dtype=x.dtype)
+    bits = torch.empty((N, H // 2, W // 2, C // 8), device=x.device, dtype=torch.int32)
+    check(_L().cddmsl_avgpool2_fwd_bits(ptr(x), ptr(y), ptr(bits), N, H, W, C, _dt(x), stream_ptr()), "cddmsl_avgpool2_fwd_bits")
+    return y, bits
+
+
+@_timed("avgpool2_bwd")
+def avgpool2_bwd_bits(dy, in_shape, bits):
+    require_cuda(dy, bits)
+    N, H, W, C = in_shape
+    assert dy.dtype == torch.bfloat16 and dy.is_contiguous() and tuple(dy.shape) == (N, H // 2, W // 2, C)
+    assert bits.dtype == torch.int32 and bits.is_contiguous() and tuple(bits.shape) == (N, H // 2, W // 2, C // 8)
+    dx = torch.empty(in_shape, device=dy.device, dtype=dy.dtype)
+    check(_L().cddmsl_avgpool2_bwd_bits(ptr(dy), ptr(bits), ptr(dx), N, H, W, C, _dt(dy), stream_ptr()), "cddmsl_avgpool2_bwd_bits")
+    return dx
 
 
 @_timed("avgpool2_bwd")
@@ -1042,7 +1090,7 @@
 
 
 @_timed("layernorm")
-def layernorm_bwd(dy, x, gamma, mean, rstd, accumulate_into=None):
+def layernorm_bwd(dy, x, gamma, mean, rstd, accumulate_into=None, emit_bf16=False):
     require_cuda(dy, x, gamma, mean, rstd, accumulate_into)
     R, D = x.shape
     dy = dy.contiguous()
@@ -1053,6 +1101,11 @@
     else:
         assert accumulate_into.dtype == torch.float32 and accumulate_into.is_contiguous() and accumulate_into.shape == x.shape
         dx, acc = accumulate_into, 1
+    if emit_bf16:
+        dxb, did = torch.empty(x.shape, device=x.device, dtype=torch.bfloat16), c_int(0)
+        check(_L().cddmsl_layernorm_bwd_emit(ptr(dy), ptr(x), ptr(gamma), ptr(mean), ptr(rstd), ptr(dx), ptr(dxb), R, D, acc, _dt(dy),
+                                             ctypes.byref(did), stream_ptr()), "cddmsl_layernorm_bwd_emit")
+        return dx, (dxb if did.value else None)
     check(_L().cddmsl_layernorm_bwd(ptr(dy), ptr(x), ptr(gamma), ptr(mean), ptr(rstd), ptr(dx), R, D, acc, _dt(dy), stream_ptr()),
           "cddmsl_layernorm_bwd")
     return dx
diff --git a/cddmsl_amd/layers.py b/cddmsl_amd/layers.py
--- a/cddmsl_amd/layers.py
+++ b/cddmsl_amd/layers.py
@@ -306,6 +306,27 @@
     return torch.cat([hip.weight_prep(_ohwi(w.detach()), None, dtype, True, False)[0] for w in weights], dim=0)
 
 
+_BF16_OF = {}
+
+
+def _bf16_key(g):
+    return (g.data_ptr(), g.numel(), g.device)
+
+
+def _register_bf16(g, gb):
+    _BF16_OF.clear()
+    if gb is not None:
+        _BF16_OF[_bf16_key(g)] = (g, g._version, gb)
+
+
+def bf16_of(g):
+    if _BF16_OF and g.dtype == torch.float32 and g.is_contiguous():
+        e = _BF16_OF.pop(_bf16_key(g), None)
+        if e is not None and e[0]._version == e[1] and g._version == e[1]:
+            return e[2].view(g.shape)
+    return g.to(torch.bfloat16)
+
+
 class ConvFn(torch.autograd.Function):
 
     @staticmethod
@@ -329,7 +350,7 @@
         if relu:
             dy = hip.relu_bwd(dy, y if y.dtype == T else y.to(T))
         elif dy.dtype != T:
-            dy = dy.to(T)
+            dy = bf16_of(dy) if T == torch.bfloat16 else dy.to(T)
         w = ctx.pw.param
         if train_w:
             if f8:
@@ -377,7 +398,7 @@
         M = h.shape[2]
         g = dy.contiguous()
         if g.dtype != T:
-            g = g.to(T)
+            g = bf16_of(g) if T == torch.bfloat16 else g.to(T)
         _, w2d = ctx.pw[1].get(T, need_dgrad=True)
         _, w1d = ctx.pw[0].get(T, need_dgrad=True)
         dh = hip.conv_fwd(g.view(1, 1, M, -1), w2d, relu_mask=h)
@@ -455,6 +476,12 @@
         self.pw = tuple(None if w is None else PreparedWeight(w, b[0], frozen) for w, b in zip(self.w, self.bn))
 
 
+def _pool_bits_wanted(bp, o2):
+    if os.environ.get("CDDMSL_POOL_MASK_BITS", "1") == "0" or o2.dtype != torch.bfloat16 or o2.shape[-1] % 8:
+        return False
+    return not (bp.fp8 and _fp8_dgrad_wanted(bp.pw[1], o2.shape, 1, True))
+
+
 def _block_forward(x, bp, save, px_given=None, next_pw=None, out_spec=None):
     (s1, b1), (s2, b2), (s3, b3), bnd = bp.bn
     pool = bp.stride > 1
@@ -466,7 +493,11 @@
     e8o2 = fp8_act_slot(bp.pw[2]).emit() if save and not pool and _fp8_wgrad1x1_wanted(bp.pw[2], M2, f8) else None
     o2 = conv_fwd_auto(o1, bp.pw[1], s2, b2, f8, emit8=e8o2, relu=True, pad=1)
     o2_8 = _fp8_made_for(o2, bp.pw[2]) if e8o2 is not None else None
-    p2 = hip.avgpool2_fwd(o2) if pool else o2
+    o2_shape, bits = tuple(o2.shape), None
+    if pool and save and _pool_bits_wanted(bp, o2):
+        p2, bits = hip.avgpool2_fwd_bits(o2)
+    else:
+        p2 = hip.avgpool2_fwd(o2) if pool else o2
     if pool and px_given is not None and tuple(px_given.shape) == (x.shape[0], x.shape[1] // 2, x.shape[2] // 2, x.shape[3]):
         px = px_given
     else:
@@ -477,10 +508,11 @@
         idn = x
     out_shape = (p2.shape[0], p2.shape[1], p2.shape[2], _ohwi(bp.w[2]).shape[0])
     out = conv_fwd_auto(p2, bp.pw[2], s3, b3, f8, emit8=fp8_emit_for(next_pw, out_shape, 0, f8), residual=idn, relu=True, out_spec=out_spec)
-    return out, ((o1, o2, p2 if pool else None, px if pool else None, (x8, _fp8_made_for(o1, bp.pw[1]) if f8 else None, o2_8)) if save else None)
-
-
-def _block_backward(gs, x, o1, o2, p2, px, bp, need_dx, mask_x, prev_bp=None, c8=(None, None, None)):
+    return out, ((o1, o2 if bits is None else bits, p2 if pool else None, px if pool else None,
+                  (x8, _fp8_made_for(o1, bp.pw[1]) if f8 else None, o2_8), o2_shape) if save else None)
+
+
+def _block_backward(gs, x, o1, o2, p2, px, bp, need_dx, mask_x, prev_bp=None, c8=(None, None, None), o2_shape=None):
     T = x.dtype
     (s1, _), (s2, _), (s3, _), bnd = bp.bn
     pool = bp.stride > 1
@@ -490,7 +522,9 @@
     gs_slot = fp8_slot_of(bp, "_fp8_gs") if f8 else None
     d2_slot = fp8_slot_of(bp.pw[1], "_fp8_g") if f8 else None
     x8, o1_8, o2_8 = c8
-    M2 = o2.shape[0] * o2.shape[1] * o2.shape[2]
+    o2_bits = o2.dtype == torch.int32
+    o2_shape = tuple(o2.shape) if o2_shape is None else tuple(o2_shape)
+    M2 = o2_shape[0] * o2_shape[1] * o2_shape[2]
     if o2_8 is not None and not pool:
         wgrad_auto(o2, gs, bp.pw[2], s3, 0, _ohwi(_grad_buf(w3p)), f8, o2_8, gs_slot, taps_only=False)
     else:
@@ -498,9 +532,12 @@
     d1_slot = fp8_slot_of(bp.pw[0], "_fp8_g") if f8 and x8 is not None and _fp8_wgrad1x1_wanted(bp.pw[0], M2, f8) else None
     if pool:
         dp2 = dgrad_auto(gs, bp.pw[2], f8, gs_slot)
-        dpre2 = hip.avgpool2_bwd(dp2, tuple(o2.shape), mask=o2, emit8=d2_slot.emit() if f8 and _fp8_dgrad_wanted(bp.pw[1], o2.shape, 1, f8) else None)
+        if o2_bits:
+            dpre2 = hip.avgpool2_bwd_bits(dp2, o2_shape, o2)
+        else:
+            dpre2 = hip.avgpool2_bwd(dp2, o2_shape, mask=o2, emit8=d2_slot.emit() if f8 and _fp8_dgrad_wanted(bp.pw[1], o2_shape, 1, f8) else None)
     else:
-        e8 = d2_slot.emit() if f8 and _fp8_dgrad_wanted(bp.pw[1], o2.shape, 1, f8) else None
+        e8 = d2_slot.emit() if f8 and _fp8_dgrad_wanted(bp.pw[1], o2_shape, 1, f8) else None
         dpre2 = dgrad_auto(gs, bp.pw[2], f8, gs_slot, emit8=e8, relu_mask=o2)
     dpre1 = dgrad_auto(dpre2, bp.pw[1], f8, d2_slot, pad=1, relu_mask=o1, emit8=d1_slot.emit() if d1_slot is not None else None)
     wgrad_auto(o1, dpre2, bp.pw[1], s2, 1, _ohwi(_grad_buf(w2p)), f8, o1_8, d2_slot)
@@ -531,14 +568,15 @@
     @staticmethod
     def forward(ctx, x, anchor, blocks, out_grad_premasked=False, px0=None, out_spec=None):
         ctx.out_grad_premasked = out_grad_premasked
-        saved, o1_8s = [x], []
+        saved, o1_8s, o2_shapes = [x], [], []
         cur = x
         for bi, bp in enumerate(blocks):
             cur, mids = _block_forward(cur, bp, True, px0 if bi == 0 else None, blocks[bi + 1].pw[0] if bi + 1 < len(blocks) else None,
                                        out_spec if bi + 1 == len(blocks) else None)
             saved += [mids[0], mids[1], mids[2], mids[3], cur]
             o1_8s += list(mids[4])
-        ctx.blocks = blocks
+            o2_shapes.append(mids[5])
+        ctx.blocks, ctx.o2_shapes = blocks, o2_shapes
         ctx.save_for_backward(*saved, *o1_8s)
         return cur
 
@@ -551,7 +589,7 @@
         for i in range(len(blocks) - 1, -1, -1):
             x, o1, o2, p2, px = saved[5 * i: 5 * i + 5]
             gs = _block_backward(gs, x, o1, o2, p2, px, blocks[i], need_dx or i > 0, mask_x=i > 0, prev_bp=blocks[i - 1] if i > 0 else None,
-                                 c8=tuple(o1_8s[3 * i: 3 * i + 3]))
+                                 c8=tuple(o1_8s[3 * i: 3 * i + 3]), o2_shape=ctx.o2_shapes[i])
         return gs, None, None, None, None, None
 
 
@@ -635,7 +673,7 @@
     return K * (out_size // 2) ** 2 > N * H * W
 
 
-def _roi_block0_forward(feat, rois, bp, out_size, scale, sr, extra, next_pw=None, on_map=None):
+def _roi_block0_forward(feat, rois, bp, out_size, scale, sr, extra, next_pw=None, on_map=None, save=False):
     T = feat.dtype
     (s1, b1), (s2, b2), (s3, b3), bnd = bp.bn
     w1, _ = bp.pw[0].get(T, False)
@@ -666,12 +704,16 @@
         if idn is None:
             px[K:].copy_(hip.avgpool2_fwd(extra))
     o2 = conv_fwd_auto(o1, bp.pw[1], s2, b2, f8, relu=True, pad=1)
-    p2 = hip.avgpool2_fwd(o2)
+    o2_shape = tuple(o2.shape)
+    if save and _pool_bits_wanted(bp, o2):
+        p2, o2 = hip.avgpool2_fwd_bits(o2)
+    else:
+        p2 = hip.avgpool2_fwd(o2)
     if idn is None:
         idn = conv_fwd_auto(px, bp.pw[3], bnd[0], bnd[1], f8)
     out_shape = (p2.shape[0], p2.shape[1], p2.shape[2], _ohwi(bp.w[2]).shape[0])
     out = conv_fwd_auto(p2, bp.pw[2], s3, b3, f8, emit8=fp8_emit_for(next_pw, out_shape, 0, f8), residual=idn, relu=True)
-    return o1, o2, p2, px, out, (_fp8_made_for(o1, bp.pw[1]) if f8 else None)
+    return o1, o2, p2, px, out, (_fp8_made_for(o1, bp.pw[1]) if f8 else None), o2_shape
 
 
 class RoIStageFn(torch.autograd.Function):
@@ -681,12 +723,14 @@
         feat = feat.contiguous()
         nxt = lambda i: blocks[i + 1].pw[0] if i + 1 < len(blocks) else None
         on_map = roi_downsample_on_map(rois.shape[0], out_size, feat.shape[0], feat.shape[1], feat.shape[2])
-        o1, o2, p2, px, cur, o1_8 = _roi_block0_forward(feat, rois, blocks[0], out_size, scale, sr, extra, nxt(0), on_map)
-        saved, o1_8s = [feat, rois, roi_start, extra, o1, o2, p2, px, cur], [None, o1_8, None]
+        o1, o2, p2, px, cur, o1_8, o2_shape = _roi_block0_forward(feat, rois, blocks[0], out_size, scale, sr, extra, nxt(0), on_map, save=True)
+        saved, o1_8s, o2_shapes = [feat, rois, roi_start, extra, o1, o2, p2, px, cur], [None, o1_8, None], [o2_shape]
         for bi, bp in enumerate(blocks[1:], start=1):
             cur, mids = _block_forward(cur, bp, True, None, nxt(bi))
             saved += [mids[0], mids[1], mids[2], mids[3], cur]
             o1_8s += list(mids[4])
+            o2_shapes.append(mids[5])
+        ctx.o2_shapes = o2_shapes
         ctx.blocks, ctx.meta = blocks, (out_size, scale, sr, out_grad_premasked, on_map)
         ctx.save_for_backward(*saved, *o1_8s)
         return cur
@@ -701,9 +745,11 @@
         gs = g.contiguous() if premasked else hip.relu_bwd(g.contiguous(), st[-1])
         for i in range(len(blocks) - 1, 0, -1):
             o1, o2, p2, px = st[5 * i: 5 * i + 4]
-            gs = _block_backward(gs, st[5 * i - 1], o1, o2, p2, px, blocks[i], True, mask_x=True, prev_bp=blocks[i - 1], c8=tuple(o1_8s[3 * i: 3 * i + 3]))
+            gs = _block_backward(gs, st[5 * i - 1], o1, o2, p2, px, blocks[i], True, mask_x=True, prev_bp=blocks[i - 1], c8=tuple(o1_8s[3 * i: 3 * i + 3]),
+                                 o2_shape=ctx.o2_shapes[i])
         bp = blocks[0]
         o1, o2, p2, px = st[0:4]
+        o2_shape = ctx.o2_shapes[0]
         T = o1.dtype
         (s1, _), (s2, _), (s3, _), bnd = bp.bn
         w1p, w2p, w3p, wdp = bp.w
@@ -713,8 +759,11 @@
         gs_slot = fp8_slot_of(bp, "_fp8_gs") if f8 else None
         d2_slot = fp8_slot_of(bp.pw[1], "_fp8_g") if f8 else None
         hip.conv_wgrad(p2, gs, shp(w3p), s3, out=_ohwi(_grad_buf(w3p)))
-        e8 = d2_slot.emit() if f8 and _fp8_dgrad_wanted(bp.pw[1], o2.shape, 1, f8) else None
-        dpre2 = hip.avgpool2_bwd(dgrad_auto(gs, bp.pw[2], f8, gs_slot), tuple(o2.shape), mask=o2, emit8=e8)
+        if o2.dtype == torch.int32:
+            dpre2 = hip.avgpool2_bwd_bits(dgrad_auto(gs, bp.pw[2], f8, gs_slot), o2_shape, o2)
+        else:
+            e8 = d2_slot.emit() if f8 and _fp8_dgrad_wanted(bp.pw[1], o2_shape, 1, f8) else None
+            dpre2 = hip.avgpool2_bwd(dgrad_auto(gs, bp.pw[2], f8, gs_slot), o2_shape, mask=o2, emit8=e8)
         dpre1 = dgrad_auto(dpre2, bp.pw[1], f8, d2_slot, pad=1, relu_mask=o1)
         wgrad_auto(o1, dpre2, bp.pw[1], s2, 1, _ohwi(_grad_buf(w2p)), f8, o1_8s[1], d2_slot)
         N, H, W, C = feat.shape
@@ -1001,16 +1050,26 @@
         x = x.contiguous()
         y, mean, rstd = hip.layernorm_fwd(x, gamma, beta, out_dtype)
         ctx.save_for_backward(x, gamma, mean, rstd)
+        ctx.emit = out_dtype == torch.bfloat16
         return y, x.view_as(x)
 
     @staticmethod
     def backward(ctx, dy, dskip):
         x, gamma, mean, rstd = ctx.saved_tensors
+        emit = ctx.emit and os.environ.get("CDDMSL_LN_EMIT_BF16", "1") != "0"
         if dskip is None:
+            if emit and dy is not None:
+                dx, dxb = hip.layernorm_bwd(dy, x, gamma, mean, rstd, emit_bf16=True)
+                _register_bf16(dx, dxb)
+                return dx, None, None, None
             return hip.layernorm_bwd(dy, x, gamma, mean, rstd), None, None, None
         acc = dskip.contiguous()
         if dy is None:
             return acc, None, None, None
+        if emit:
+            dx, dxb = hip.layernorm_bwd(dy, x, gamma, mean, rstd, accumulate_into=acc, emit_bf16=True)
+            _register_bf16(dx, dxb)
+            return dx, None, None, None
         return hip.layernorm_bwd(dy, x, gamma, mean, rstd, accumulate_into=acc), None, None, None
 
 
diff --git a/cddmsl_amd/modeling/backbone.py b/cddmsl_amd/modeling/backbone.py
--- a/cddmsl_amd/modeling/backbone.py
+++ b/cddmsl_amd/modeling/backbone.py
@@ -1,3 +1,4 @@
+import os
 from collections import OrderedDict
 
 import torch
@@ -184,6 +185,8 @@
         (s1, b1), (s2, b2), (s3, b3) = self.bn1.affine(), self.bn2.affine(), self.bn3.affine()
         x = hip.conv_fwd(x, w1, s1, b1, relu=True, stride=2, pad=1)
         x = hip.conv_fwd(x, w2, s2, b2, relu=True, pad=1)
+        if x.dtype == torch.bfloat16 and tuple(w3.shape) == (64, 3, 3, 32) and os.environ.get("CDDMSL_STEM_POOL", "1") != "0":
+            return hip.conv3x3_pool_fwd(x, w3, s3, b3)
         x = hip.conv_fwd(x, w3, s3, b3, relu=True, pad=1)
         return hip.avgpool2_fwd(x)
 
diff --git a/include/cddmsl_hip.h b/include/cddmsl_hip.h
--- a/include/cddmsl_hip.h
+++ b/include/cddmsl_hip.h
@@ -11,6 +11,8 @@
 int cddmsl_conv_fwd(const void* x, const void* w, void* y, const float* scale, const float* bias, const void* residual,
                     const void* relu_mask, int Nimg, int Hi, int Wi, int Cin, int Cout, int KH, int KW, int stride, int pad,
                     int pool, int ldy, int ldr, int ldm, int relu, int out_f32, int dtype, void* stream);
+int cddmsl_conv3x3_pool_fwd(const void* x, const void* w, void* y, const float* scale, const float* bias, const void* relu_mask,
+                            int Nimg, int Hi, int Wi, int Cin, int Cout, int stride, int dtype, void* stream);
 int cddmsl_bottleneck64_ok(int Nimg, int H, int W, int dtype);
 int cddmsl_bottleneck64_fwd(const void* o1, const void* w2, const float* s2, const float* b2, const void* w3, const float* s3,
                             const float* b3, const void* residual, const void* x0, const void* wd, const float* sd,
@@ -137,6 +139,8 @@
                          float eps, int dtype, void* stream);
 int cddmsl_layernorm_bwd(const void* dy, const float* x, const float* gamma, const float* mean, const float* rstd, float* dx,
                          long R, int D, int accumulate, int dtype, void* stream);
+int cddmsl_layernorm_bwd_emit(const void* dy, const float* x, const float* gamma, const float* mean, const float* rstd, float* dx,
+                              void* dx_bf16, long R, int D, int accumulate, int dtype, int* emitted, void* stream);
 int cddmsl_focal_ce_fwd(const float* logits, const long* target, float* row_loss, float* probs, long R, int C, float gamma,
                         int bg_class, float bg_weight, void* stream);
 int cddmsl_focal_ce_bwd(const float* logits, const long* target, const float* probs, const float* gscale, float* dlogits, long R,
@@ -161,6 +165,8 @@
 int cddmsl_avgpool2_fwd(const void* x, void* y, int N, int H, int W, int C, int dtype, void* stream);
 int cddmsl_avgpool2_bwd(const void* dy, const void* mask, const void* add, void* dx, int N, int H, int W, int C, int dtype,
                         void* stream);
+int cddmsl_avgpool2_fwd_bits(const void* x, void* y, void* bits, int N, int H, int W, int C, int dtype, void* stream);
+int cddmsl_avgpool2_bwd_bits(const void* dy, const void* bits, void* dx, int N, int H, int W, int C, int dtype, void* stream);
 int cddmsl_avgpool2_bwd_q8(const void* dy, const void* mask, const void* add, void* dx, int N, int H, int W, int C, void* y8,
                            const float* q8, float* amax8, void* stream);
 int cddmsl_maxpool3s2_fwd(const void* x, void* y, int N, int H, int W, int C, int dtype, void* stream);
```
